# iris-ua/iris_lama

Hardware: AMD Instinct MI355X
Metric: particle-scans/sec (higher is better)
Workload: dtype f64; 1 GPU; PFSlam2D 30 particles, 1080-beam synthetic corridor log (SURVEY.md 8(d)), res 0.05 m, patch 32, l2_max 0.5, GN+Cauchy(0.15), seed 42; particles=30, beams=1080, parallelism=particle-shard x1

## Files before the change

iris_lama_amd/csrc/lama_dev.h:

```cpp
#pragma once
#include <hip/hip_runtime.h>
#include <stdint.h>
#include <cstddef>
#include <type_traits>

#ifdef LAMA_WIDE_DM
#define lama_dev lama_dev_wide
#endif

#include "lama_heap.h"

#ifdef LAMA_WAVE_SIM
#define LAMA_LOCKSTEP() ((void)__ballot(true))
#else
#define LAMA_LOCKSTEP() ((void)0)
#endif

namespace lama_dev {

#ifdef LAMA_WIDE_DM
typedef uint32_t sv_t;
constexpr uint32_t SV_VALID = 0x80000000u;
constexpr uint32_t SV_QUEUED = 0x40000000u;
constexpr uint32_t SV_SQMASK = 0x3FFFFFFFu;
constexpr int SV_VALID_BIT = 31;
constexpr uint32_t MAX_OFFSET_CELLS = 255;
#else
typedef uint16_t sv_t;
constexpr uint16_t SV_VALID = 0x8000;
constexpr uint16_t SV_QUEUED = 0x4000;
constexpr uint16_t SV_SQMASK = 0x3FFF;
constexpr int SV_VALID_BIT = 15;
constexpr uint32_t MAX_OFFSET_CELLS = 127;
#endif
constexpr uint32_t SV_BYTES = (uint32_t)sizeof(sv_t);
constexpr uint32_t SV_PATCH_BYTES = 1024u * SV_BYTES;

constexpr int ERR_WINDOW = 1;
constexpr int ERR_DM_CAP = 2;
constexpr int ERR_OCC_CAP = 4;
constexpr int ERR_QUEUE = 8;
constexpr int ERR_NUMERIC = 16;
constexpr int ERR_CLEAN_ABORT = 32;

struct Affine {
    double R[3][3];
    double t[3];
};

struct PartRec {
    uint32_t home, dm_cap, occ_cap, r0;
    sv_t* dm_sv; uint32_t* dm_obs; uint64_t* dm_mask;
    uint32_t* occ; uint64_t* occ_mask; uint64_t* occ_hit;
    int32_t* rev;
    uint64_t r1;
};

struct DevParams {
    uint32_t P;
    uint32_t W;
    uint32_t WC;
    uint32_t wx0, wy0;
    uint32_t qcap;
    const PartRec* part;
    uint32_t max_sqdist;
    uint32_t max_iter;
    double scale, off, resolution, maxdist, meas_sigma;
    double trunc_ray, trunc_range;
    int16_t* dm_dir;
    int16_t* occ_dir;
    int32_t* counts;
    double* poses;
    uint64_t* q_lower;
    uint64_t* q_raise;
    uint32_t* qsizes;
    uint32_t* slow;
    uint32_t* slow_list;
    uint32_t* slow_n;
    uint8_t* heavy;
    const uint32_t* elist;
    const uint32_t* elist_n;
    const uint8_t* early;
    uint32_t lane;
    uint64_t* act;
    uint32_t* act_count;
    uint32_t act_cap;
    uint64_t* stats;
    int32_t* err;
    uint64_t* dbg;
    uint32_t* guard;
    uint32_t guard_r;
    uint32_t occ_policy, ray_rule;
    uint32_t strategy;
    double lo_miss, lo_hit, lo_min, lo_max;
    uint32_t ghosts;
};

constexpr int ARG_BLOCK = 16;
struct PoseTable { double v[4 * ARG_BLOCK]; };
struct TfTable { double v[12 * ARG_BLOCK]; };
struct NoTable {};

struct PV {
    int16_t* dm_dir; int16_t* occ_dir;
    sv_t* dm_sv; uint32_t* dm_obs; uint64_t* dm_mask;
    uint32_t* occ; uint64_t* occ_mask; uint64_t* occ_hit;
    int32_t* counts; int32_t* rev;
    uint32_t dm_cap, occ_cap;
};
#ifdef LAMA_WAVE_SIM
__device__ inline uint32_t part_u32(const uint32_t* q) { return *q; }
__device__ inline uint64_t part_u64(const uint64_t* q) { return *q; }
#else
__device__ inline uint32_t part_u32(const uint32_t* q)
{
    return (uint32_t)__builtin_amdgcn_readfirstlane((int)__hip_atomic_load(q, __ATOMIC_RELAXED, __HIP_MEMORY_SCOPE_AGENT));
}
__device__ inline uint64_t part_u64(const uint64_t* q)
{
    const uint64_t v = __hip_atomic_load(q, __ATOMIC_RELAXED, __HIP_MEMORY_SCOPE_AGENT);
    const uint32_t lo = (uint32_t)__builtin_amdgcn_readfirstlane((int)(uint32_t)v), hi = (uint32_t)__builtin_amdgcn_readfirstlane((int)(uint32_t)(v >> 32));
    return ((uint64_t)hi << 32) | lo;
}
#endif
#if defined(LAMA_KC_PROBE) && !defined(LAMA_WAVE_SIM)
__device__ uint32_t g_kc_n;
__device__ uint64_t g_kc_ev[64][8];
__device__ __noinline__ void kc_probe(const DevParams& prm, int p)
{
    const uint64_t* q = reinterpret_cast<const uint64_t*>(prm.part + p);
#if LAMA_KC_PROBE == 2
    __builtin_amdgcn_s_dcache_inv();
#endif
    const unsigned long long act = __ballot(1);
    const bool rec = (int)(threadIdx.x & 63u) == __ffsll((long long)act) - 1;
    for (int k = 0; k < 9; ++k) {
        const uint64_t* qa = q + k;
        const uint64_t ua = (uint64_t)qa;
        const uint64_t sa = ((uint64_t)(uint32_t)__builtin_amdgcn_readfirstlane((int)(uint32_t)(ua >> 32)) << 32) | (uint32_t)__builtin_amdgcn_readfirstlane((int)(uint32_t)ua);
// ... 418 lines not shown
```

iris_lama_amd/csrc/lama_hip.hip:

```cpp
#include "../../include/lama_hip.h"

#include <hip/hip_runtime.h>

#include <algorithm>
#include <cmath>
#include <cstdio>
#include <cstdlib>
#include <cstring>
#include <map>
#include <memory>
#include <mutex>
#include <string>
#include <vector>

#include "lama_kernels.h"
#include "lama_pgo.h"
#include "lama_pgo_pcg.h"
#include "lama_map_build.h"
#include "lama_raster.h"
#include "lama_frontier.h"
#include "lama_raycast_query.h"
#include "lama_match_batch.h"
#include "lama_correlative.h"
#include "../host/pgo_pattern.hpp"
// ... 150 lines not shown
    size_t ev_used = 0;
    bool initialised = false;
    bool poisoned = false;
    bool dm_deleted = false;

    uint32_t P = 0, W = 0, WC = 0, wx0 = 0, wy0 = 0;
    uint32_t max_sqdist = 0;
    double scale = 0, off = 0;

    MapStore ms;
    std::vector<RegionAlloc> ra_dm, ra_occ;
    std::vector<HostPart> h_part;
    DevBuf<PartRec> d_part;
    PinVec<PartRec> h_part_stage;
    PinVec<CloneJob> h_jobs; DevBuf<CloneJob> d_jobs;
    PinVec<ZeroJob> h_zjobs; DevBuf<ZeroJob> d_zjobs;
    uint32_t floor_dm = 128, floor_occ = 128;
    PinVec<uint32_t> h_guard;
    uint64_t clone_bytes = 0;
    double* d_poses = nullptr;
    DevBuf<uint64_t> d_qlower, d_qraise;
    uint64_t* d_stats = nullptr;
    DevBuf<uint32_t> d_qsizes;
    DevBuf<uint64_t> d_dbg;
    DevBuf<uint32_t> d_slow;
    DevBuf<uint32_t> d_slow_list; uint32_t* d_slow_n = nullptr;
    DevBuf<uint8_t> d_heavy;
    DevBuf<uint8_t> d_early; DevBuf<uint32_t> d_elist;
    Stream stream3; Event ev_alloc, ev_go, ev_early;
    bool early_ok = false;
    uint32_t early_candidates = 0;
    std::vector<double> h_ll; bool ll_valid = false;
    PinVec<uint32_t> h_hlist; DevBuf<uint32_t> d_hlist;
    uint32_t early_on = 1;
    uint32_t early_min_count = 1024;
    Stream stream2; Event ev_route, ev_heavy;
    uint32_t route_min_count = 64, route_min_events = 48, route_percent = 150, route_cap = 64;
    bool route_forced = false; uint32_t num_cus = 256;
    bool debug_tail = false, debug_window = false;
    uint32_t big_stage_pad = 0;
    DevBuf<uint64_t> d_act; DevBuf<uint32_t> d_act_count;
    DevBuf<lama_dev::RayRec> d_rrec; DevBuf<uint64_t> d_rbbox; DevBuf<lama_dev::RayChunk> d_rchunk;
    int32_t* d_err = nullptr;
    DevBuf<double> d_pts; uint32_t last_n = 0;
    PinVec<uint64_t> h_stats;
    PinVec<double> h_tfs, h_pts;
    PinVec<int32_t> h_err;
    PinVec<uint32_t> h_slow_n;
    DevBuf<double> d_tfs;
    double* d_loglik = nullptr; int32_t* d_iters = nullptr;
    DevBuf<uint8_t> d_results;
    size_t results_bytes = 0, status_off = 0, status_bytes = 0;
    PinVec<uint8_t> h_status;
    PinVec<uint8_t> h_results;
    DevBuf<int32_t> d_oldcounts;
    DevBuf<double> d_mb_pts, d_mb_tfs; DevBuf<uint32_t> d_mb_offs; DevBuf<lama_dev::MbRay> d_mb_rays;
    DevBuf<uint32_t> d_mb_table, d_mb_off, d_mb_list, d_mb_bins; DevBuf<int32_t> d_mb_slot; DevBuf<uint64_t> d_mb_meta;
    PinVec<double> h_mb_tfs; PinVec<uint32_t> h_mb_offs; PinVec<uint64_t> h_mb_meta;
    DevBuf<uint8_t> d_raster; PinVec<uint8_t> h_raster;
    DevBuf<lama_dev::FrontierRec> d_frontier_rec;
    DevBuf<double> d_rq_in; DevBuf<uint8_t> d_rq_out; PinVec<double> h_rq_tfs;
    DevBuf<double> d_bposes, d_bout;
    DevBuf<double> d_msb_f64; DevBuf<uint32_t> d_msb_u32;
    PinVec<double> h_msb_f64; PinVec<uint32_t> h_msb_u32;
    DevBuf<double> d_cs_tfs; DevBuf<uint64_t> d_cs_best;
    PinVec<double> h_cs_tfs;

    double scan_reach = 0.0;
    uint32_t visit_bound = 0;
    DevBuf<uint32_t> d_scalar;
    DevBuf<lama_dev::ShipDesc> d_ship_desc; DevBuf<uint8_t> d_ship_heads;
    PinVec<lama_dev::ShipDesc> h_ship_desc; PinVec<uint8_t> h_ship_heads;
    uint32_t* d_guard = nullptr;
    Affine last_mtf; uint32_t last_first = 0, last_count = 0;
    bool last_guarded = false;
    int recover_depth = 0;
    int64_t mbx0 = 0, mbx1 = 0, mby0 = 0, mby1 = 0; bool mb_valid = false;
    bool unguarded_retry = false;
    uint32_t saved_visit_bound = 0; lama_hip_counters saved_ctr;
    bool pending_maps = false;
    StepGroup grp[MAX_STEP_GROUPS];
    Stream stream4;
    uint32_t step_groups = 1;
    uint32_t groups_ran = 0;
    std::vector<int32_t> deferred_idx; bool resample_deferred = false;
    bool groups_busy = false;
    PinVec<double> h_pts2; uint32_t scan_slot = 0;
    std::vector<uint64_t> h_chain;
    bool chain_dirty = false;
    double step_ms[3] = {0, 0, 0}; bool step_ms_any[3] = {false, false, false};
    PinVec<double> h_poses;
    PinVec<int32_t> h_counts;
    lama_hip_counters ctr;

    ~lama_hip_ctx()
    {
        (void)hipSetDevice(cfg.device);
        if (stream) (void)hipStreamSynchronize(stream);
        for (StepGroup& g : grp) if (g.s) (void)hipStreamSynchronize(g.s);
    }
};

namespace {

int32_t hip_fail(lama_hip_ctx* ctx, hipError_t e, const char* what)
{
    ctx->error = std::string(what) + ": " + hipGetErrorString(e);
    (void)hipStreamSynchronize(ctx->stream);
    if (ctx->groups_busy) for (StepGroup& g : ctx->grp) if (g.s) (void)hipStreamSynchronize(g.s);
    return LAMA_HIP_E_HIP;
}
#define HIPCHK(ctx, call)                                                                              \
    do {                                                                                               \
        const hipError_t e_ = (call);                                                                  \
        if (e_ != hipSuccess) return hip_fail((ctx), e_, #call);                                       \
    } while (0)

int32_t fail(lama_hip_ctx* ctx, int32_t code, const std::string& msg)
{
    ctx->error = msg;
    return code;
}

Affine moving_tf(const double* origin3, const double* q)
{
    Affine a;
    const double w = q ? q[0] : 1.0, x = q ? q[1] : 0.0, y = q ? q[2] : 0.0, z = q ? q[3] : 0.0;
    const double tx = 2.0 * x, ty = 2.0 * y, tz = 2.0 * z;
    const double twx = tx * w, twy = ty * w, twz = tz * w;
    const double txx = tx * x, txy = ty * x, txz = tz * x;
    const double tyy = ty * y, tyz = tz * y, tzz = tz * z;
    a.R[0][0] = 1.0 - (tyy + tzz); a.R[0][1] = txy - twz;         a.R[0][2] = txz + twy;
    a.R[1][0] = txy + twz;         a.R[1][1] = 1.0 - (txx + tzz); a.R[1][2] = tyz - twx;
    a.R[2][0] = txz - twy;         a.R[2][1] = tyz + twx;         a.R[2][2] = 1.0 - (txx + tyy);
    for (int i = 0; i < 3; ++i) a.t[i] = origin3 ? origin3[i] : 0.0;
    return a;
}

void host_scan_tf(const double* pose4, const Affine& m, double* out12)
{
    const double theta = std::atan2(pose4[1], pose4[0]);
    const double sn = std::sin(theta), cs = std::cos(theta);
    const double F[3][3] = {{cs, 0.0 - sn, 0.0}, {sn, cs, 0.0}, {0.0, 0.0, (1.0 - cs) + cs}};
    const double ft[3] = {pose4[2], pose4[3], 0.0};
    for (int i = 0; i < 3; ++i) {
        for (int j = 0; j < 3; ++j) out12[3 * i + j] = (F[i][0] * m.R[0][j] + F[i][1] * m.R[1][j]) + F[i][2] * m.R[2][j];
        out12[9 + i] = ((F[i][0] * m.t[0] + F[i][1] * m.t[1]) + F[i][2] * m.t[2]) + ft[i];
    }
}

uint32_t guard_radius(const lama_hip_ctx* c)
{
    const uint32_t r = (uint32_t)std::ceil(std::sqrt((double)c->max_sqdist));
    return ((c->dm_deleted ? 2u * r + 1u : r) + 1u + 31u) / 32u;
}

DevParams make_params(const lama_hip_ctx* c)
{
    DevParams p;
    p.P = c->P; p.W = c->W; p.WC = c->WC; p.wx0 = c->wx0; p.wy0 = c->wy0;
    p.qcap = c->cfg.queue_capacity; p.part = c->d_part;
    p.max_sqdist = c->max_sqdist; p.max_iter = c->cfg.max_iter;
    p.scale = c->scale; p.off = c->off; p.resolution = c->cfg.resolution;
    p.maxdist = std::sqrt((double)c->max_sqdist) * c->cfg.resolution;
    p.meas_sigma = c->cfg.meas_sigma;
    p.trunc_ray = c->cfg.truncated_ray; p.trunc_range = c->cfg.truncated_range;
// ... 18 lines not shown
}

int32_t wait_for_groups(lama_hip_ctx* c)
{
    if (!c->groups_busy) return LAMA_HIP_OK;
    for (StepGroup& g : c->grp)
        if (g.count) { const hipError_t e = hipStreamSynchronize(g.s); if (e != hipSuccess) { c->error = std::string("hipStreamSynchronize(group stream): ") + hipGetErrorString(e); return LAMA_HIP_E_HIP; } }
    return LAMA_HIP_OK;
}

bool scan_reach2(const double* pts, size_t n, bool strict, double& r2)
{
    double nan_acc = r2 = 0.0;
    for (size_t i = 0; i < n; ++i) { const double d2 = pts[3 * i] * pts[3 * i] + pts[3 * i + 1] * pts[3 * i + 1] + pts[3 * i + 2] * pts[3 * i + 2]; r2 = std::max(r2, d2); nan_acc += d2 * 0.0; }
    return std::isfinite(r2) && (!strict || nan_acc == 0.0);
}

int32_t upload_scan(lama_hip_ctx* c, const double* pts, uint32_t n)
{
    if (!pts) {
        if (c->last_n == 0 || n != c->last_n) return fail(c, LAMA_HIP_E_INVALID, "pts == NULL but no matching scan is resident");
        return LAMA_HIP_OK;
    }
    c->last_n = n;
    HIPCHK(c, c->d_pts.grow((size_t)3 * n, (size_t)3 * 2048));
    c->h_pts.resize((size_t)3 * n);
    std::memcpy(c->h_pts.data(), pts, sizeof(double) * 3 * n);
    double r2 = 0.0;
    if (!scan_reach2(pts, n, false, r2)) { c->last_n = 0; return fail(c, LAMA_HIP_E_INVALID, "the scan holds a non-finite point (filter NaN / inf ranges before the update, as iris_lama_ros does)"); }
    c->scan_reach = std::sqrt(r2);
    HIPCHK(c, hipMemcpyAsync(c->d_pts, c->h_pts.data(), sizeof(double) * 3 * n, hipMemcpyHostToDevice, c->stream));
    return LAMA_HIP_OK;
}

int32_t ensure_batch(lama_hip_ctx* c, size_t entries, size_t floor = 0)
{
    if (entries <= c->d_bout.n) return LAMA_HIP_OK;
    c->d_bposes.reset(); c->d_bout.reset();
    const size_t cap = std::max(entries, floor);
    HIPCHK(c, c->d_bposes.alloc(4 * cap));
    HIPCHK(c, c->d_bout.alloc(cap));
    return LAMA_HIP_OK;
}

void resolve_timers(lama_hip_ctx* c);
int32_t grow_arenas(lama_hip_ctx* c, uint32_t first, uint32_t count);
int32_t recover_update(lama_hip_ctx* c, int32_t e);
int32_t run_update_maps(lama_hip_ctx* c, uint32_t n, const Affine& mtf, uint32_t first, uint32_t count);
int32_t permute_particles(lama_hip_ctx* c, const int32_t* idx);

int32_t clamp_counts(lama_hip_ctx* c, bool fetch)
{
    if (fetch) HIPCHK(c, hipMemcpyAsync(c->h_counts.data(), c->ms.counts, sizeof(int32_t) * 2 * c->P, hipMemcpyDeviceToHost, c->stream));
    HIPCHK(c, hipStreamSynchronize(c->stream));
    bool clamped = false;
    for (uint32_t p = 0; p < c->P; ++p) {
        const HostPart& hp = c->h_part[p];
        if ((uint32_t)c->h_counts[2 * p] > hp.dm_cap) { c->h_counts[2 * p] = (int32_t)hp.dm_cap; clamped = true; }
        if ((uint32_t)c->h_counts[2 * p + 1] > hp.occ_cap) { c->h_counts[2 * p + 1] = (int32_t)hp.occ_cap; clamped = true; }
    }
    if (clamped) {
        HIPCHK(c, hipMemcpyAsync(c->ms.counts, c->h_counts.data(), sizeof(int32_t) * 2 * c->P, hipMemcpyHostToDevice, c->stream));
        HIPCHK(c, hipStreamSynchronize(c->stream));
    }
    return LAMA_HIP_OK;
}

int32_t device_error_result(lama_hip_ctx* c, int32_t e)
{
    if (e & ERR_WINDOW) return fail(c, LAMA_HIP_E_WINDOW, "a map cell fell outside the device window (the mapped area is wider than 1016 patches)");
    if (e & ERR_DM_CAP) return fail(c, LAMA_HIP_E_CAPACITY, "a particle's distance map exceeds 32767 patches (or the device is out of memory)");
    if (e & ERR_OCC_CAP) return fail(c, LAMA_HIP_E_CAPACITY, "a particle's occupancy map exceeds 32767 patches (or the device is out of memory)");
    if (e & ERR_QUEUE) return fail(c, LAMA_HIP_E_CAPACITY, "brushfire queue full (raise cfg.queue_capacity)");
    return fail(c, LAMA_HIP_E_NUMERIC, "unit complex number is (near) zero (SophusException in the reference)");
}

struct StatusView {
    const uint8_t *err, *slow_n, *stats, *guard, *counts; uint32_t base, n;
    int32_t error() const { int32_t e; std::memcpy(&e, err, sizeof(e)); return e; }
};

void apply_update_status(lama_hip_ctx* c, const StatusView& v, uint32_t first, uint32_t count, uint64_t* chain)
{
    uint32_t sn[5]; std::memcpy(sn, v.slow_n, sizeof(sn));
    c->ctr.brushfire_handovers += sn[0]; c->ctr.replay_handovers += sn[1] + sn[3]; c->ctr.brushfire_routed += sn[2] + sn[4]; c->ctr.brushfire_early += sn[4];
    c->early_candidates = sn[2] + sn[4];
    c->h_guard.resize(c->P);
    std::memcpy(&c->h_guard[v.base], v.guard, sizeof(uint32_t) * v.n);
    std::memcpy(&c->h_counts[2 * (size_t)v.base], v.counts, sizeof(int32_t) * 2 * v.n);
    if (v.error() != 0) return;
    for (uint32_t p = first; p < first + count; ++p) {
        uint64_t st[4]; std::memcpy(st, v.stats + sizeof(st) * (p - v.base), sizeof(st));
        c->ctr.ray_cells += st[2]; c->ctr.bf_cells += st[3]; if (chain) chain[p] = st[3];
    }
}

void refresh_patch_totals(lama_hip_ctx* c)
{
    c->ctr.dm_patches = c->ctr.occ_patches = 0;
    for (uint32_t p = 0; p < c->P; ++p) { c->ctr.dm_patches += c->h_counts[2 * p]; c->ctr.occ_patches += c->h_counts[2 * p + 1]; }
}

int32_t check_device_errors(lama_hip_ctx* c, bool maps = false, bool match = false, bool err_in_results = false)
{
    c->h_err.resize(1);
    int32_t& e = c->h_err[0] = 0;
    if (maps || match) c->h_stats.resize((size_t)c->P * 4);
    if (maps) {
        c->h_status.resize(c->status_bytes); c->h_slow_n.resize(5);
        HIPCHK(c, hipMemcpyAsync(c->h_status.data(), c->d_results + c->status_off, c->status_bytes, hipMemcpyDeviceToHost, c->stream));
    } else {
        if (match) {
            HIPCHK(c, hipMemcpyAsync(c->h_counts.data(), c->ms.counts, sizeof(int32_t) * 2 * c->P, hipMemcpyDeviceToHost, c->stream));
            HIPCHK(c, hipMemcpyAsync(c->h_stats.data(), c->d_stats, sizeof(uint64_t) * c->h_stats.size(), hipMemcpyDeviceToHost, c->stream));
        }
        if (!err_in_results) HIPCHK(c, hipMemcpyAsync(&e, c->d_err, sizeof(e), hipMemcpyDeviceToHost, c->stream));
    }
    HIPCHK(c, hipStreamSynchronize(c->stream));
    if (maps) {
        const uint8_t* const b = c->h_status.data(), * const sn = b + ((const uint8_t*)c->d_slow_n - (c->d_results + c->status_off));
        const StatusView v{b, sn, sn + 32, sn + 32 + 32 * (size_t)c->P, sn + 32 + 40 * (size_t)c->P, 0u, c->P};
        e = v.error();
        std::memcpy(c->h_slow_n.data(), v.slow_n, 5 * sizeof(uint32_t));
        std::memcpy(c->h_stats.data(), v.stats, sizeof(uint64_t) * 4 * c->P);
        apply_update_status(c, v, c->last_first, c->last_count, nullptr);
    }
    if (err_in_results) std::memcpy(&e, c->h_results.data() + ((const uint8_t*)c->d_err - c->d_results), sizeof(e));
    resolve_timers(c);
    if (e != 0) {
        HIPCHK(c, hipMemsetAsync(c->d_err, 0, sizeof(int32_t), c->stream));
        if (maps && (e & ERR_CLEAN_ABORT) && (e & (ERR_DM_CAP | ERR_OCC_CAP)) && !(e & ERR_WINDOW) && c->last_guarded && c->recover_depth < 10) {
            const int32_t rr = recover_update(c, e);
            if (rr != LAMA_HIP_E_CAPACITY) return rr;
        }
        if (e & (ERR_DM_CAP | ERR_OCC_CAP)) { const int32_t rcl = clamp_counts(c, !(maps || match)); if (rcl) return rcl; }
        return device_error_result(c, e);
    }
    if (match) for (uint32_t p = 0; p < c->P; ++p) { c->ctr.gn_iterations += c->h_stats[4 * p]; c->ctr.gn_evals += c->h_stats[4 * p + 1]; }
    if (maps || match) refresh_patch_totals(c);
    if (!maps) return LAMA_HIP_OK;
    uint64_t mx = 0, sum = 0; uint32_t arg = 0;
    for (uint32_t p = c->last_first; p < c->last_first + c->last_count; ++p) { const uint64_t v = c->h_stats[4 * p + 3]; sum += v; if (v > mx) { mx = v; arg = p; } }
    c->ctr.bf_longest_chain_sum += mx; c->ctr.bf_longest_chain_last = mx;
    if (c->debug_tail) {
        uint32_t rank = 0; double ll = 0, mean_ll = 0;
        if (c->h_results.size() >= c->results_bytes && c->P > 1) {
            const double* L = reinterpret_cast<const double*>(c->h_results.data() + sizeof(double) * 4 * c->P);
            ll = L[arg];
            for (uint32_t p = 0; p < c->P; ++p) { rank += L[p] < ll ? 1u : 0u; mean_ll += L[p]; }
            mean_ll /= c->P;
        }
        std::fprintf(stderr, "brushfire pops: mean %.0f max %llu (particle %u) handovers %u brushfire %.3f ms; log-lik of that particle %.1f (pool mean %.1f), rank %u of %u\n", (double)sum / c->P, (unsigned long long)mx, arg, c->h_slow_n[0], c->ctr.ms_brushfire, ll, mean_ll, rank, c->P);
    }
    return grow_arenas(c, 0, c->P);
}

constexpr uint32_t MAX_PATCHES = 32767u;

static uint32_t round_up32(uint32_t v) { return (v + 31u) / 32u * 32u; }

static uint32_t want_capacity(uint32_t floor_cap, uint32_t count, uint32_t extra)
{
    const uint32_t head = std::max<uint32_t>(std::max<uint32_t>(32u, count / 4u), extra);
    return std::min<uint32_t>(MAX_PATCHES, std::max<uint32_t>(floor_cap, round_up32(count + head)));
}

static PartRec dev_part(const lama_hip_ctx* c, const HostPart& h)
{
// ... 328 lines not shown
    const dim3 grid((unsigned)P, (unsigned)((std::max(WW, nWW) + 255) / 256));
    int16_t* const to_dm = nd[0]; int16_t* const to_occ = nd[1];
    hipLaunchKernelGGL(k_shift_window, grid, dim3(256), 0, c->stream, c->ms.dm_dir, to_dm, c->W, newW, dx, dy, WW, nWW, c->d_err);
    hipLaunchKernelGGL(k_shift_window, grid, dim3(256), 0, c->stream, c->ms.occ_dir, to_occ, c->W, newW, dx, dy, WW, nWW, c->d_err);
    {
        hipError_t e = hipGetLastError();
        if (e == hipSuccess) e = hipStreamSynchronize(c->stream);
        if (e != hipSuccess) return hip_fail(c, e, "k_shift_window");
    }
    c->ms.dm_dir.swap(nd[0]); c->ms.occ_dir.swap(nd[1]);
    if (newW != c->W) {
        c->W = newW; c->WC = newW * 32; c->cfg.window_patches = newW;
        c->ctr.window_growths += 1;
    }
    c->wx0 = (uint32_t)(nox * 32); c->wy0 = (uint32_t)(noy * 32);
    c->ctr.window_shifts += 1;
    c->ctr.window_patches = c->W;
    return LAMA_HIP_OK;
}

int32_t ensure_window(lama_hip_ctx* c, int64_t x0, int64_t x1, int64_t y0, int64_t y1)
{
    if (!c->mb_valid) { c->mbx0 = x0; c->mbx1 = x1; c->mby0 = y0; c->mby1 = y1; c->mb_valid = true; }
    else { c->mbx0 = std::min(c->mbx0, x0); c->mbx1 = std::max(c->mbx1, x1); c->mby0 = std::min(c->mby0, y0); c->mby1 = std::max(c->mby1, y1); }
    const int64_t ox = c->wx0 >> 5, oy = c->wy0 >> 5, W = c->W;
    if (c->debug_window) std::fprintf(stderr, "ensure_window: box x [%ld, %ld] y [%ld, %ld] mapped x [%ld, %ld] y [%ld, %ld] window x [%ld, %ld) y [%ld, %ld)\n", (long)x0, (long)x1, (long)y0, (long)y1, (long)c->mbx0, (long)c->mbx1, (long)c->mby0, (long)c->mby1, (long)ox, (long)(ox + W), (long)oy, (long)(oy + W));
    if (c->mbx0 >= ox && c->mbx1 < ox + W && c->mby0 >= oy && c->mby1 < oy + W) return LAMA_HIP_OK;
    const int64_t span = std::max(c->mbx1 - c->mbx0 + 1, c->mby1 - c->mby0 + 1);
    int64_t newW = W;
    if (span > W) newW = std::min<int64_t>(LAMA_HIP_MAX_WINDOW, std::max<int64_t>((span + 8 + 7) / 8 * 8, (W + W / 2 + 7) / 8 * 8));
    int64_t hx0 = c->mbx0, hx1 = c->mbx1, hy0 = c->mby0, hy1 = c->mby1;
    if (span > newW) { hx0 = x0; hx1 = x1; hy0 = y0; hy1 = y1; if (x1 - x0 + 1 > newW || y1 - y0 + 1 > newW) return LAMA_HIP_OK; }
    auto place = [&](int64_t o, int64_t lo, int64_t hi) {
        const int64_t a = hi - newW + 1, b = lo;
        int64_t no = std::min(std::max(o, a), b);
        if (no > o) no = std::min(no + 4, b); else if (no < o) no = std::max(no - 4, a);
        return no;
    };
    const int64_t nox = c->initialised ? place(ox, hx0, hx1) : (hx0 + hx1 + 1) / 2 - newW / 2;
    const int64_t noy = c->initialised ? place(oy, hy0, hy1) : (hy0 + hy1 + 1) / 2 - newW / 2;
    return regrid_window(c, (uint32_t)newW, nox, noy);
}

int32_t start_without_first_scan(lama_hip_ctx* c)
{
    if (c->initialised) return LAMA_HIP_OK;
    for (uint32_t p = 0; p < c->P; ++p) { c->h_poses[4 * p] = 1.0; c->h_poses[4 * p + 1] = 0.0; c->h_poses[4 * p + 2] = 0.0; c->h_poses[4 * p + 3] = 0.0; }
    HIPCHK(c, hipMemcpyAsync(c->d_poses, c->h_poses.data(), sizeof(double) * 4 * c->P, hipMemcpyHostToDevice, c->stream));
    c->initialised = true;
    return LAMA_HIP_OK;
}

int32_t fit_window(lama_hip_ctx* c, const Affine& mtf, uint32_t first, uint32_t count)
{
    double far = c->scan_reach;
    if (c->cfg.ray_rule == 0 && c->cfg.truncated_range > 0.0) far = std::min(far, c->cfg.truncated_range);
    const uint32_t guard_r = guard_radius(c);
    const double reach = far + std::sqrt(mtf.t[0] * mtf.t[0] + mtf.t[1] * mtf.t[1]) + (double)(guard_r + 1u) * 32.0 * c->cfg.resolution;
    double xlo = 1e300, xhi = -1e300, ylo = 1e300, yhi = -1e300;
    for (uint32_t p = first; p < first + count; ++p) {
        const double x = c->h_poses[4 * p + 2], y = c->h_poses[4 * p + 3];
        xlo = std::min(xlo, x - reach); xhi = std::max(xhi, x + reach);
        ylo = std::min(ylo, y - reach); yhi = std::max(yhi, y + reach);
    }
    auto patch = [&](double w) { return (int64_t)std::floor((c->scale * w + c->off) / 32.0); };
    return ensure_window(c, patch(xlo), patch(xhi), patch(ylo), patch(yhi));
}

static uint32_t route_places(const lama_hip_ctx* c, uint32_t count)
{
    const uint32_t slots = c->num_cus * 12u;
    if (c->route_forced || count >= slots) return c->route_cap;
    return std::min<uint32_t>(c->route_cap, std::max<uint32_t>(8u, (slots - count) / 7u));
}

struct UpdatePlan {
    hipStream_t s = nullptr; const double* d_pts = nullptr; uint32_t n = 0, first = 0, count = 0;
    DevParams prm;
    lama_dev::TfTable tab = lama_dev::TfTable(); bool tf_by_value = false;
    StepGroup* timers = nullptr;
    bool sequential = false, guarded = true, canon = false, two_waves = false, route = false, early_lane = false;
    bool prev_routed = false; uint32_t host_n = 0;
    uint32_t route_places = 0; unsigned gy = 0, resume_grid = 0; bool replay_large = true;
};

static bool parallel_raycast_ruled_out(const lama_hip_ctx* c, uint32_t n)
{
    return c->cfg.sequential_raycast == 1 || c->cfg.occupancy_policy == 1 || c->cfg.ray_rule == 1 || n > 4096u || (uint64_t)n + 4096u > c->cfg.active_capacity;
}

UpdatePlan plan_update(lama_hip_ctx* c, uint32_t n, uint32_t first, uint32_t count, bool wrap_sequential, StepGroup* g = nullptr)
{
    UpdatePlan u;
    u.n = n; u.first = first; u.count = count; u.timers = g; u.tf_by_value = g && count <= (uint32_t)lama_dev::ARG_BLOCK;
    u.s = g ? g->s : (hipStream_t)c->stream; u.d_pts = g ? (const double*)g->d_pts : (const double*)c->d_pts; u.prm = g ? group_params(c, *g) : make_params(c);
    u.two_waves = c->cfg.brushfire_waves == 2 || (c->cfg.brushfire_waves == 0 && count <= BF_TW_MAX_PARTICLES);
    u.gy = count <= 64 ? 128u : (count >= 1024 ? 8u : 32u);
#ifdef LAMA_WAVE_SIM
    u.gy = 4u;
#endif
    u.replay_large = count <= 512; u.resume_grid = std::min<unsigned>(count, 256u);
    if (g) return u;
    u.sequential = parallel_raycast_ruled_out(c, n) || wrap_sequential;
    u.guarded = c->cfg.ray_rule == 0;
    u.canon = c->cfg.brushfire_mode == 1;
    u.route = u.two_waves && count >= c->route_min_count && c->route_cap > 0; u.route_places = route_places(c, count);
    if (u.sequential || !(c->early_on && u.two_waves && !u.canon && first == 0 && count == c->P &&
                          count >= std::max<uint32_t>(c->route_min_count, c->early_min_count) && c->route_cap > 0)) return u;
    if (c->ll_valid) {
        double mean = 0; for (uint32_t p = 0; p < c->P; ++p) mean += c->h_ll[p]; mean /= c->P;
        const double lim = 2.5 * std::min(mean, 0.0) - 5.0;
        std::vector<std::pair<double, uint32_t>> cand;
        for (uint32_t p = 0; p < c->P; ++p) if (c->h_ll[p] < lim) cand.emplace_back(c->h_ll[p], p);
        if (cand.size() > u.route_places) { std::partial_sort(cand.begin(), cand.begin() + u.route_places, cand.end()); cand.resize(u.route_places); }
        c->h_hlist.resize(256);
        for (auto& e : cand) c->h_hlist[u.host_n++] = e.second;
    }
    u.prev_routed = c->early_ok && c->early_candidates > 0; u.early_lane = u.host_n > 0 || u.prev_routed;
    return u;
}

int32_t wrap_guard_probe(lama_hip_ctx* c, uint32_t n, int64_t& bound)
{
    if (parallel_raycast_ruled_out(c, n) || (uint64_t)c->visit_bound + n < 65536u) return LAMA_HIP_OK;
    uint32_t m = 0;
    if (c->initialised) {
        const DevParams prm = make_params(c);
        (void)hipMemsetAsync(c->d_scalar, 0, sizeof(uint32_t), c->stream);
        hipLaunchKernelGGL(k_occ_max_visited, dim3(c->P), dim3(256), 0, c->stream, prm, c->d_scalar);
        HIPCHK(c, hipMemcpyAsync(&m, c->d_scalar, sizeof(uint32_t), hipMemcpyDeviceToHost, c->stream));
        HIPCHK(c, hipStreamSynchronize(c->stream));
    }
    bound = m;
    return LAMA_HIP_OK;
}

int32_t pregrow_unguarded(lama_hip_ctx* c, uint32_t first, uint32_t count)
{
    if (c->cfg.ray_rule == 0) return LAMA_HIP_OK;
    const double rp = c->scan_reach / (32.0 * c->cfg.resolution) + 2.5;
    const uint32_t bound = (uint32_t)std::min(32767.0, std::ceil(3.1416 * rp * rp));
    std::vector<CapRequest> reqs;
    for (uint32_t p = first; p < first + count; ++p) {
        const HostPart& pr = c->h_part[p];
        const uint32_t nd = std::min<uint32_t>(MAX_PATCHES, round_up32((uint32_t)c->h_counts[2 * p] + bound)), no = std::min<uint32_t>(MAX_PATCHES, round_up32((uint32_t)c->h_counts[2 * p + 1] + bound));
        if (nd > pr.dm_cap || no > pr.occ_cap) reqs.push_back(CapRequest{p, std::max(nd, pr.dm_cap), std::max(no, pr.occ_cap)});
    }
    return reqs.empty() ? LAMA_HIP_OK : set_capacities(c, reqs);
}

void note_update_begin(lama_hip_ctx* c, const Affine& mtf, const UpdatePlan& u, int64_t probed)
{
    c->last_mtf = mtf; c->last_first = u.first; c->last_count = u.count; c->last_guarded = u.guarded;
    if (c->recover_depth == 0) { c->saved_visit_bound = c->visit_bound; c->saved_ctr = c->ctr; }
    if (probed >= 0) { c->visit_bound = (uint32_t)probed; if (u.sequential) c->ctr.wrap_guard_scans += 1; }
    c->visit_bound = (uint32_t)std::min<uint64_t>((uint64_t)c->visit_bound + u.n, 65535u);
    if (u.sequential) c->ctr.sequential_raycast_scans += 1; else c->ctr.parallel_raycast_scans += 1;
    c->early_ok = u.route && u.first == 0 && u.count == c->P;
}

int32_t stage_scan_tfs(lama_hip_ctx* c, const Affine& mtf, uint32_t first, uint32_t count, hipStream_t s, lama_dev::TfTable* tab)
{
    PinVec<double>& tfs = c->h_tfs; tfs.resize((size_t)c->P * 12);
    for (uint32_t p = first; p < first + count; ++p) host_scan_tf(&c->h_poses[4 * p], mtf, &tfs[12 * (size_t)p]);
    if (tab) std::memcpy(tab->v, &tfs[12 * (size_t)first], sizeof(double) * 12 * count);
    else HIPCHK(c, hipMemcpyAsync(c->d_tfs + 12 * (size_t)first, &tfs[12 * (size_t)first], sizeof(double) * 12 * count, hipMemcpyHostToDevice, s));
    return LAMA_HIP_OK;
}

static unsigned xcd_grid(const lama_hip_ctx* c, uint32_t first, uint32_t count)
{
    return first + count == c->P ? (count + 7u) / 8u * 8u : count;
}

template <class Tab>
int32_t launch_allocation_phase(lama_hip_ctx* c, const UpdatePlan& u, int alloc_only, const Tab& tab)
{
    const uint32_t n = u.n, first = u.first, count = u.count;
    const double* const d_tfs = u.tf_by_value ? nullptr : (const double*)c->d_tfs;
    const size_t need = (size_t)c->P * n;
    if (need > c->d_rrec.n) {
        c->d_rrec.reset(); c->d_rbbox.reset(); c->d_rchunk.reset();
        hipError_t e = c->d_rrec.alloc(need);
        if (e == hipSuccess) e = c->d_rbbox.alloc(need);
        if (e == hipSuccess) e = c->d_rchunk.alloc((size_t)c->P * ((n + 63) / 64));
        if (e != hipSuccess) { c->d_rrec.reset(); return hip_fail(c, e, "ray buffers"); }
    }
    const dim3 hits_grid(xcd_grid(c, first, count), (n + 255) / 256);
    hipLaunchKernelGGL(k_ray_hits<Tab>, hits_grid, dim3(256), 0, u.s, u.prm, u.d_pts, (int)n, d_tfs, (int)first,
                       (lama_dev::RayRec*)c->d_rrec, (uint64_t*)c->d_rbbox, alloc_only, (lama_dev::RayChunk*)c->d_rchunk, tab);
    const int rw_seg = count <= 64 ? 4 : 1;
    hipLaunchKernelGGL(k_ray_alloc_walk, dim3(xcd_grid(c, first, count), (n * rw_seg + 255) / 256), dim3(256), 0, u.s, u.prm, (const lama_dev::RayRec*)c->d_rrec, (int)n, (int)first, rw_seg);
    double far = c->scan_reach;
    if (c->cfg.truncated_range > 0.0) far = std::min(far, c->cfg.truncated_range);
    const int reach_cells = (int)std::ceil(far * c->scale) + 2;
    uint32_t row0 = 0, row1 = c->W - 1;
    if (c->mb_valid) {
        const int64_t oy = c->wy0 >> 5, W = c->W;
        const int64_t lo = std::min(std::max(c->mby0 - oy, (int64_t)0), W - 1), hi = std::min(std::max(c->mby1 - oy, (int64_t)0), W - 1);
        if (hi >= lo) { row0 = (uint32_t)lo; row1 = (uint32_t)hi; }
    }
    hipLaunchKernelGGL(k_occ_reverse_dir<Tab>, dim3(count), dim3(256), 0, u.s, u.prm, (int)first, d_tfs, reach_cells, c->unguarded_retry ? 1 : 0, row0, row1, tab);
    return LAMA_HIP_OK;
}
int32_t launch_allocation_phase(lama_hip_ctx* c, const UpdatePlan& u, int alloc_only) { return u.tf_by_value ? launch_allocation_phase(c, u, alloc_only, u.tab) : launch_allocation_phase(c, u, alloc_only, lama_dev::NoTable()); }

int32_t launch_early_lane(lama_hip_ctx* c, const UpdatePlan& u)
{
    DevParams pe = u.prm; pe.elist = c->d_elist; pe.elist_n = c->d_slow_n + 4; pe.lane = 1;
    hipLaunchKernelGGL(k_ray_patches, dim3(u.route_places, 128u), dim3(256), 0, c->stream, pe, (const lama_dev::RayRec*)c->d_rrec,
                       (const uint64_t*)c->d_rbbox, (const lama_dev::RayChunk*)c->d_rchunk, (int)u.n, 0);
    hipLaunchKernelGGL((k_ray_replay<RP_SORT_SMALL, RP_SORT_SMALL, false, RP_BLOCK_LARGE>), dim3(u.route_places), dim3(RP_BLOCK_LARGE), 0, c->stream, pe, 0);
    hipLaunchKernelGGL((k_ray_replay<8192, 8192, true, RP_BLOCK_LARGE>), dim3(u.route_places), dim3(RP_BLOCK_LARGE), 0, c->stream, pe, 0);
    HIPCHK(c, hipEventRecord(c->ev_alloc, c->stream));
    HIPCHK(c, hipStreamWaitEvent(c->stream3, c->ev_alloc, 0));
    hipLaunchKernelGGL(k_mark_early, dim3(1), dim3(64), 0, c->stream3, pe);
    HIPCHK(c, hipEventRecord(c->ev_go, c->stream3));
    hipLaunchKernelGGL((k_brushfire<LQ_BIG, RQ_BIG, true, true>), dim3(u.route_places), dim3(2 * UM_BLOCK), c->big_stage_pad, c->stream3, pe, 0, 2);
    HIPCHK(c, hipEventRecord(c->ev_early, c->stream3));
    HIPCHK(c, hipStreamWaitEvent(c->stream, c->ev_go, 0));
    return LAMA_HIP_OK;
}

int32_t launch_parallel_raycast(lama_hip_ctx* c, const UpdatePlan& u)
{
    const int first = (int)u.first; const uint32_t host_n = u.host_n;
    if (u.early_lane) {
        if (host_n) HIPCHK(c, hipMemcpyAsync(c->d_hlist, c->h_hlist.data(), sizeof(uint32_t) * host_n, hipMemcpyHostToDevice, c->stream));
        hipLaunchKernelGGL(k_early_list, dim3(1), dim3(256), 0, c->stream, u.prev_routed ? (const uint8_t*)c->d_heavy : (const uint8_t*)nullptr,
                           (const uint32_t*)c->d_hlist, host_n, c->d_early, c->d_elist, c->d_slow_n + 4, (int)c->P, u.route_places);
    }
    { const int32_t ra = launch_allocation_phase(c, u, 0); if (ra) return ra; }
    DevParams prm = u.prm;
    if (u.early_lane) { const int32_t re = launch_early_lane(c, u); if (re) return re; prm.early = c->d_early; }
    hipLaunchKernelGGL(k_ray_patches, dim3(xcd_grid(c, u.first, u.count), u.gy), dim3(256), 0, u.s, prm, (const lama_dev::RayRec*)c->d_rrec,
                       (const uint64_t*)c->d_rbbox, (const lama_dev::RayChunk*)c->d_rchunk, (int)u.n, first);
    if (u.replay_large) {
        hipLaunchKernelGGL((k_ray_replay<RP_SORT_SMALL, RP_SORT_SMALL, false, RP_BLOCK_LARGE>), dim3(u.count), dim3(RP_BLOCK_LARGE), 0, u.s, prm, first);
        hipLaunchKernelGGL((k_ray_replay<8192, 8192, true, RP_BLOCK_LARGE>), dim3(u.resume_grid), dim3(RP_BLOCK_LARGE), 0, u.s, prm, first);
    } else {
        hipLaunchKernelGGL((k_ray_replay<RP_SORT_SMALL, RP_SORT_SMALL, false, RP_BLOCK_SMALL>), dim3(u.count), dim3(RP_BLOCK_SMALL), 0, u.s, prm, first);
        hipLaunchKernelGGL((k_ray_replay<8192, 8192, true, RP_BLOCK_SMALL>), dim3(u.resume_grid), dim3(RP_BLOCK_SMALL), 0, u.s, prm, first);
    }
    return LAMA_HIP_OK;
}

int32_t launch_brushfire(lama_hip_ctx* c, const UpdatePlan& u)
{
    const int first = (int)u.first;
    DevParams prm = u.prm; if (u.early_lane) prm.early = c->d_early;
    if (u.canon) hipLaunchKernelGGL(k_brushfire_canon, dim3(u.count), dim3(CN_BLOCK), 0, u.s, prm, first);
    if (u.route) {
        prm.heavy = c->d_heavy;
        hipLaunchKernelGGL(k_bf_route, dim3(1), dim3(256), 0, c->stream, prm, first, (int)u.count, c->route_min_events, c->route_percent, u.route_places);
        HIPCHK(c, hipEventRecord(c->ev_route, c->stream));
        hipLaunchKernelGGL((k_brushfire<LQ_BIG, RQ_BIG, true, true>), dim3(u.route_places), dim3(2 * UM_BLOCK), 0, c->stream, prm, first, 1);
        HIPCHK(c, hipStreamWaitEvent(c->stream2, c->ev_route, 0));
        hipLaunchKernelGGL((k_brushfire<LQ_SMALL, RQ_SMALL, false, true>), dim3(u.count), dim3(2 * UM_BLOCK), 0, c->stream2, prm, first, 0);
        HIPCHK(c, hipEventRecord(c->ev_heavy, c->stream2));
        HIPCHK(c, hipStreamWaitEvent(c->stream, c->ev_heavy, 0));
    } else if (u.two_waves) hipLaunchKernelGGL((k_brushfire<LQ_SMALL, RQ_SMALL, false, true>), dim3(u.count), dim3(2 * UM_BLOCK), 0, u.s, prm, first, 0);
    else hipLaunchKernelGGL((k_brushfire<LQ_SMALL, RQ_SMALL, false, false>), dim3(u.count), dim3(UM_BLOCK), 0, u.s, prm, first, 0);
    if (u.two_waves) hipLaunchKernelGGL((k_brushfire<LQ_BIG, RQ_BIG, true, true>), dim3(u.resume_grid), dim3(2 * UM_BLOCK), 0, u.s, prm, first, 0);
    else hipLaunchKernelGGL((k_brushfire<LQ_BIG, RQ_BIG, true, false>), dim3(u.resume_grid), dim3(UM_BLOCK), 0, u.s, prm, first, 0);
    if (u.early_lane) HIPCHK(c, hipStreamWaitEvent(c->stream, c->ev_early, 0));
    hipLaunchKernelGGL(k_brushfire_slow, dim3(u.count), dim3(UM_BLOCK), 0, u.s, prm, first);
    return LAMA_HIP_OK;
}

int32_t launch_update(lama_hip_ctx* c, const UpdatePlan& u, Timer& ray_timer)
{
    int32_t rc = !u.sequential ? launch_parallel_raycast(c, u) : u.guarded ? launch_allocation_phase(c, u, 1) : LAMA_HIP_OK;
    if (rc) return rc;
    if (u.sequential) hipLaunchKernelGGL(k_raycast, dim3(u.count), dim3(UM_BLOCK), 0, u.s, u.prm, u.d_pts, (int)u.n, c->d_tfs, (int)u.first);
    ray_timer.stop();
    HIPCHK(c, hipGetLastError());
    Timer t = Timer::of_update(c, u.timers, 2);
    c->ctr.brushfire_mode = c->cfg.brushfire_mode; c->ctr.brushfire_waves = u.two_waves ? 2u : 1u;
    rc = launch_brushfire(c, u);
    if (rc) return rc;
    t.stop();
    HIPCHK(c, hipGetLastError());
    return LAMA_HIP_OK;
}

int32_t run_update_maps(lama_hip_ctx* c, uint32_t n, const Affine& mtf, uint32_t first, uint32_t count)
{
    int32_t rc = fit_window(c, mtf, first, count);
    if (rc == LAMA_HIP_OK) rc = stage_scan_tfs(c, mtf, first, count, c->stream, nullptr);
    if (rc) return rc;
    Timer t = Timer::of_update(c, nullptr, 1);
    const bool whole = first == 0 && count == c->P;
    (void)hipMemsetAsync(c->d_slow_n, 0, whole ? 32 + sizeof(uint64_t) * 4 * c->P : 32, c->stream);
    if (!whole) (void)hipMemsetAsync(c->d_stats + 4 * (size_t)first, 0, sizeof(uint64_t) * 4 * count, c->stream);
    int64_t probed = -1; rc = wrap_guard_probe(c, n, probed);
    if (rc == LAMA_HIP_OK) rc = pregrow_unguarded(c, first, count);
    if (rc) return rc;
    const UpdatePlan u = plan_update(c, n, first, count, probed >= 0 && (uint64_t)probed + n >= 65536u);
    note_update_begin(c, mtf, u, probed);
    return launch_update(c, u, t);
}


int32_t permute_particles(lama_hip_ctx* c, const int32_t* idx)
{
    const uint32_t P = c->P;
    std::vector<uint8_t> taken(P, 0);
    std::vector<HostPart> np(P);
    std::vector<int32_t> nc(2 * (size_t)P);
    std::vector<double> npose(4 * (size_t)P);
    std::vector<uint32_t> clones;
    for (uint32_t i = 0; i < P; ++i) {
        const uint32_t j = (uint32_t)idx[i];
        std::memcpy(&npose[4 * i], &c->h_poses[4 * j], sizeof(double) * 4);
        nc[2 * i] = c->h_counts[2 * j]; nc[2 * i + 1] = c->h_counts[2 * j + 1];
        if (!taken[j]) { taken[j] = 1; np[i] = c->h_part[j]; } else clones.push_back(i);
    }
    std::vector<uint32_t> dead;
    for (uint32_t j = 0; j < P; ++j) if (!taken[j]) dead.push_back(j);
    c->h_jobs.resize(0); c->h_zjobs.resize(0);
    c->clone_bytes = 0;
    const size_t WW = (size_t)c->W * c->W;
    uint32_t dir_off16 = 0, dir_n16 = (uint32_t)(WW * 2 / 16);
    {
        const int64_t oy = c->wy0 >> 5, W = c->W;
        if (c->mb_valid) {
            const int64_t lo = std::min(std::max(c->mby0 - oy, (int64_t)0), W - 1), hi = std::min(std::max(c->mby1 - oy, (int64_t)0), W - 1);
            if (hi >= lo) { dir_off16 = (uint32_t)(lo * W * 2 / 16); dir_n16 = (uint32_t)((hi - lo + 1) * W * 2 / 16); }
        }
    }
    struct Slot { bool keep_dm, keep_occ; HostPart rec; int32_t odm, oocc; };
    std::vector<Slot> slots(dead.size());
    for (size_t k = 0; k < dead.size(); ++k) {
        const uint32_t d = dead[k], i = clones[k], j = (uint32_t)idx[i];
        const HostPart& dr = c->h_part[d];
        const HostPart& sr = c->h_part[j];
        Slot sl{dr.dm_cap == sr.dm_cap, dr.occ_cap == sr.occ_cap, dr, c->h_counts[2 * d], c->h_counts[2 * d + 1]};
        void* dp[5];
        region_ptrs(c, dr, dp);
        ZeroJob z{};
        if (!sl.keep_dm) { z.ndm = sl.odm; z.d[0] = dp[0]; z.d[1] = dp[1]; z.d[2] = dp[2]; region_release(c, true, dr.dm_chunk, dr.dm_off, dr.dm_cap); }
        if (!sl.keep_occ) { z.nocc = sl.oocc; z.d[3] = dp[3]; z.d[4] = dp[4]; region_release(c, false, dr.occ_chunk, dr.occ_off, dr.occ_cap); }
        if (z.ndm || z.nocc) { c->h_zjobs.resize(c->h_zjobs.size() + 1); c->h_zjobs[c->h_zjobs.size() - 1] = z; }
        slots[k] = sl;
    }
// ... 252 lines not shown
        (cfg.window_patches & 7) || cfg.dm_patch_capacity > 32767 || cfg.occ_patch_capacity > 32767 ||
        cfg.queue_capacity < (uint32_t)LQ_BIG)
        return LAMA_HIP_E_INVALID;
    int ndev = 0;
    if (hipGetDeviceCount(&ndev) != hipSuccess || ndev <= 0 || cfg.device < 0 || cfg.device >= ndev) return LAMA_HIP_E_HIP;

    std::unique_ptr<lama_hip_ctx, Delete> owner(new lama_hip_ctx());
    lama_hip_ctx* c = owner.get();
    c->cfg = cfg;
    std::memset(&c->ctr, 0, sizeof(c->ctr));
    c->P = cfg.particles; c->W = cfg.window_patches; c->WC = c->W * 32;
    c->ctr.window_patches = c->W;
    c->debug_tail = std::getenv("LAMA_HIP_DEBUG_TAIL") != nullptr;
    c->debug_window = std::getenv("LAMA_HIP_DEBUG_WINDOW") != nullptr;
    {
        constexpr uint32_t CU_LDS = 160u * 1024u, GRAN = 1280u;
        const uint32_t used = (uint32_t)((sizeof(lama_dev::BfLds<LQ_BIG, RQ_BIG>) + GRAN - 1) / GRAN * GRAN);
        c->big_stage_pad = CU_LDS > used + 2u * GRAN ? CU_LDS - used - 2u * GRAN : 0u;
    }
    if (const char* rr = std::getenv("LAMA_HIP_BF_ROUTE")) {
        unsigned a = 0, b = 0, pc = 0, d = 0, e = 1;
        if (std::sscanf(rr, "%u,%u,%u,%u,%u", &a, &b, &pc, &d, &e) >= 4) { c->route_min_count = a; c->route_min_events = b; c->route_percent = pc; c->route_cap = std::min(d, 256u); c->early_on = e; c->early_min_count = 0; c->route_forced = true; }
    }
    c->scale = 1.0 / cfg.resolution;
    c->off = double(2642244ull >> 1) * 32.0;
    uint32_t md = (uint32_t)std::ceil(cfg.l2_max * c->scale);
    c->max_sqdist = md * md;
    if (c->max_sqdist == 0 || md > MAX_OFFSET_CELLS) return LAMA_HIP_E_INVALID;

    if (hipSetDevice(cfg.device)) return LAMA_HIP_E_HIP;
    { hipDeviceProp_t prop; if (hipGetDeviceProperties(&prop, cfg.device) == hipSuccess && prop.multiProcessorCount > 0) c->num_cus = (uint32_t)prop.multiProcessorCount; }
    if (hipStreamCreate(&c->stream.h) || hipEventCreate(&c->ev0.h) || hipEventCreate(&c->ev1.h)) return LAMA_HIP_E_HIP;
    const size_t P = c->P, WW = (size_t)c->W * c->W, dc = cfg.dm_patch_capacity, oc = cfg.occ_patch_capacity;
    {
        MapStore& m = c->ms;
        c->floor_dm = (uint32_t)dc; c->floor_occ = (uint32_t)oc;
        if (P * dc > 0xFFFFFFF0ull || P * oc > 0xFFFFFFF0ull) return LAMA_HIP_E_INVALID;
        if (m.dm_dir.alloc(P * WW) || hipMemset(m.dm_dir, 0xFF, P * WW * 2)) return LAMA_HIP_E_HIP;
        if (m.occ_dir.alloc(P * WW) || hipMemset(m.occ_dir, 0xFF, P * WW * 2)) return LAMA_HIP_E_HIP;
        if (add_chunk(c, true, (uint32_t)(P * dc)) != LAMA_HIP_OK || add_chunk(c, false, (uint32_t)(P * oc)) != LAMA_HIP_OK) return LAMA_HIP_E_HIP;
        c->ctr.pool_growths = 0;
        c->h_part.resize(P);
        for (size_t p = 0; p < P; ++p) {
            HostPart r{};
            r.home = (uint32_t)p; r.dm_cap = (uint32_t)dc; r.occ_cap = (uint32_t)oc;
            if (region_alloc(c, true, (uint32_t)dc, r.dm_chunk, r.dm_off) != LAMA_HIP_OK || region_alloc(c, false, (uint32_t)oc, r.occ_chunk, r.occ_off) != LAMA_HIP_OK) return LAMA_HIP_E_HIP;
            c->h_part[p] = r;
        }
        if (c->d_part.alloc(P)) return LAMA_HIP_E_HIP;
        if (upload_part(c) != LAMA_HIP_OK) return LAMA_HIP_E_HIP;
        if (hipStreamSynchronize(c->stream)) return LAMA_HIP_E_HIP;
    }
    c->results_bytes = P * 4 * 8 + P * 8 + P * 4 + 8;
    c->status_off = P * 4 * 8 + P * 8 + P * 4;
    const size_t slow_off = (c->results_bytes + 7) / 8 * 8;
    c->status_bytes = (slow_off - c->status_off) + 32 + P * 4 * 8 + P * 2 * 4 + P * 2 * 4;
    if (c->d_results.alloc(c->status_off + c->status_bytes) || hipMemset(c->d_results, 0, c->status_off + c->status_bytes)) return LAMA_HIP_E_HIP;
    c->d_poses = reinterpret_cast<double*>(c->d_results.p);
    c->d_loglik = c->d_poses + P * 4;
    c->d_iters = reinterpret_cast<int32_t*>(c->d_loglik + P);
    c->d_err = c->d_iters + P;
    c->d_slow_n = reinterpret_cast<uint32_t*>(c->d_results + slow_off);
    c->d_stats = reinterpret_cast<uint64_t*>(c->d_results + slow_off + 32);
    c->d_guard = reinterpret_cast<uint32_t*>(c->d_stats + P * 4);
    c->ms.counts = reinterpret_cast<int32_t*>(c->d_guard + P * 2);
    if (c->d_qlower.alloc(P * (size_t)cfg.queue_capacity) || c->d_qraise.alloc(P * (size_t)cfg.queue_capacity)) return LAMA_HIP_E_HIP;
    if (c->d_qsizes.alloc(P * 2) || hipMemset(c->d_qsizes, 0, P * 2 * 4)) return LAMA_HIP_E_HIP;
    if (c->d_dbg.alloc(P * 16 + (1u << 20) / 8) || hipMemset(c->d_dbg, 0, P * 16 * 8 + (1u << 20))) return LAMA_HIP_E_HIP;
    if (c->d_slow.alloc(P) || hipMemset(c->d_slow, 0, P * 4)) return LAMA_HIP_E_HIP;
    if (c->d_slow_list.alloc(4 * P) || hipMemset(c->d_slow_list, 0, 4 * P * 4)) return LAMA_HIP_E_HIP;
    if (c->d_heavy.alloc(P) || hipMemset(c->d_heavy, 0, P)) return LAMA_HIP_E_HIP;
    if (c->d_early.alloc(P) || hipMemset(c->d_early, 0, P)) return LAMA_HIP_E_HIP;
    if (c->d_elist.alloc(256) || hipMemset(c->d_elist, 0, 256 * 4)) return LAMA_HIP_E_HIP;
    if (c->d_hlist.alloc(256) || hipMemset(c->d_hlist, 0, 256 * 4)) return LAMA_HIP_E_HIP;
    if (hipStreamCreate(&c->stream2.h) || hipStreamCreate(&c->stream3.h)) return LAMA_HIP_E_HIP;
    {
        uint32_t G = c->P < c->route_min_count ? DEFAULT_STEP_GROUPS : 1u;
        if (const char* sg = std::getenv("LAMA_HIP_STEP_GROUPS")) {
            unsigned v = 0;
            if (std::sscanf(sg, "%u", &v) == 1 && v >= 1) G = std::min<uint32_t>(v, MAX_STEP_GROUPS);
        }
        if (c->P >= c->route_min_count) G = 1;
        c->step_groups = G;
        if (G > 1) {
            if (G > 3 && hipStreamCreate(&c->stream4.h)) return LAMA_HIP_E_HIP;
            const hipStream_t ss[MAX_STEP_GROUPS] = {c->stream, c->stream2, c->stream3, c->stream4};
            uint32_t per = (uint32_t)((P + G - 1) / G);
            const uint32_t per8 = (per + 7u) / 8u * 8u;
            if ((P + per8 - 1) / per8 == G) per = per8;
            for (uint32_t k = 0; k < G; ++k) {
                StepGroup& g = c->grp[k];
                g.s = ss[k];
                g.first = (uint32_t)std::min<size_t>(P, (size_t)k * per); g.count = (uint32_t)std::min<size_t>(P, (size_t)(k + 1) * per) - g.first;
                if (g.count == 0) continue;
                const GroupPack L(g.count);
                if (g.d_words.alloc(16) || hipMemset(g.d_words, 0, 64) || g.d_slow_list.alloc(4 * P) || hipMemset(g.d_slow_list, 0, 4 * P * 4) ||
                    g.d_pack.alloc(L.bytes) || hipEventCreateWithFlags(&g.ev_match.h, hipEventDisableTiming))
                    return LAMA_HIP_E_HIP;
                g.h_pack.resize(L.bytes);
                if (cfg.profile) for (Event& e : g.tev) if (hipEventCreate(&e.h)) return LAMA_HIP_E_HIP;
            }
            c->h_chain.assign(P, 0);
        }
    }
    if (hipEventCreateWithFlags(&c->ev_alloc.h, hipEventDisableTiming) || hipEventCreateWithFlags(&c->ev_early.h, hipEventDisableTiming) ||
        hipEventCreateWithFlags(&c->ev_go.h, hipEventDisableTiming) ||
        hipEventCreateWithFlags(&c->ev_route.h, hipEventDisableTiming) || hipEventCreateWithFlags(&c->ev_heavy.h, hipEventDisableTiming))
        return LAMA_HIP_E_HIP;
    if (c->d_scalar.alloc(4) || hipMemset(c->d_scalar, 0, 16)) return LAMA_HIP_E_HIP;
    if (c->d_act.alloc(P * (size_t)cfg.active_capacity)) return LAMA_HIP_E_HIP;
    if (c->d_act_count.alloc(P) || hipMemset(c->d_act_count, 0, P * 4)) return LAMA_HIP_E_HIP;
    if (c->d_tfs.alloc(P * 12) || c->d_oldcounts.alloc(P * 2)) return LAMA_HIP_E_HIP;
    if (hipDeviceSynchronize()) return LAMA_HIP_E_HIP;
    c->h_poses.assign(P * 4, 0.0);
    c->h_counts.assign(P * 2, 0);
    *out = owner.release();
    return LAMA_HIP_OK;
}

void lama_hip_ctx_destroy(lama_hip_ctx* c) { delete c; }

int32_t lama_hip_pf_set_poses(lama_hip_ctx* c, const double* poses)
{
    if (!c || !poses) return LAMA_HIP_E_INVALID;
    ENTER(c);
    HIPCHK(c, hipSetDevice(c->cfg.device));
    std::memcpy(c->h_poses.data(), poses, sizeof(double) * 4 * c->P);
    HIPCHK(c, hipMemcpyAsync(c->d_poses, c->h_poses.data(), sizeof(double) * 4 * c->P, hipMemcpyHostToDevice, c->stream));
    return LAMA_HIP_OK;
}

int32_t lama_hip_pf_get_poses(lama_hip_ctx* c, double* poses)
{
    if (!c || !poses) return LAMA_HIP_E_INVALID;
    ENTER(c);
    std::memcpy(poses, c->h_poses.data(), sizeof(double) * 4 * c->P);
    return LAMA_HIP_OK;
}

int32_t lama_hip_pf_init(lama_hip_ctx* c, const double* pts, uint32_t n, const double* origin3, const double* quat,
                         const double* pose0)
{
    if (!c || !pts || !pose0 || n == 0) return LAMA_HIP_E_INVALID;
    ENTER(c);
    if (c->initialised) return fail(c, LAMA_HIP_E_STATE, "lama_hip_pf_init called twice");
    HIPCHK(c, hipSetDevice(c->cfg.device));
    const double mx = c->scale * pose0[2] + c->off, my = c->scale * pose0[3] + c->off;
    const uint32_t px = ((uint32_t)mx) >> 5, py = ((uint32_t)my) >> 5;
    c->wx0 = (px - c->W / 2) * 32;
    c->wy0 = (py - c->W / 2) * 32;
    for (uint32_t p = 0; p < c->P; ++p) std::memcpy(&c->h_poses[4 * p], pose0, sizeof(double) * 4);
    HIPCHK(c, hipMemcpyAsync(c->d_poses, c->h_poses.data(), sizeof(double) * 4 * c->P, hipMemcpyHostToDevice, c->stream));
    int32_t rc = upload_scan(c, pts, n);
    if (rc) return rc;
    const Affine mtf = moving_tf(origin3, quat);
    rc = run_update_maps(c, n, mtf, 0, 1);
    if (rc) return rc;
    rc = check_device_errors(c, true, false);
    if (rc) return rc;
    if (c->P > 1) {
        std::vector<int32_t> idx(c->P, 0);
        rc = permute_particles(c, idx.data());
        if (rc) return rc;
    }
    rc = check_device_errors(c, true, false);
    if (rc) return rc;
// ... 847 lines not shown
    if (iterations) *iterations = st.iters;
    if (rel_residual_sq) *rel_residual_sq = st.bb == 0.0 ? 0.0 : st.rr / st.bb;
    if (outcome) *outcome = oc;
    if (model_decrease) *model_decrease = st.model;
    if (kernel_ms) { float ms = 0; PGOCHK(g, hipEventElapsedTime(&ms, g->ev0, g->ev1)); *kernel_ms = ms; }
    return LAMA_HIP_OK;
}

int32_t lama_hip_pgo_try_solved_step(lama_hip_pgo* g, double* half_chi2, double* kernel_ms)
{
    if (!g || !half_chi2) return LAMA_HIP_E_INVALID;
    if (!g->solution_valid) {
        g->error = "lama_hip_pgo_try_solved_step: no solution of the system at the current state (call lama_hip_pgo_solve_pcg first)";
        return LAMA_HIP_E_STATE;
    }
    g->candidate_pending = false;
    PGOCHK(g, hipSetDevice(g->device));
    PgoPtrs p{g->d_cand, g->d_fi, g->d_fj, g->d_meas, g->d_sqrt, g->d_err, g->d_hoff, g->d_fdi, g->d_fdj, g->d_fg, g->d_incptr, g->d_inc,
              g->d_hdiag, g->d_b, g->d_chi};
    PGOCHK(g, hipEventRecord(g->ev0, g->stream));
    hipLaunchKernelGGL(k_pgo_retract, dim3((g->N + PGO_BLOCK - 1) / PGO_BLOCK), dim3(PGO_BLOCK), 0, g->stream, (const double*)g->d_poses,
                       (const double*)g->d_px, (double*)g->d_cand, g->N);
    if (g->robust) hipLaunchKernelGGL(k_pgo_error_robust, dim3(g->blocksF), dim3(PGO_BLOCK), 0, g->stream, p, pgo_loss_ptrs(g), (const double*)g->d_cand, g->F);
    else hipLaunchKernelGGL(k_pgo_error, dim3(g->blocksF), dim3(PGO_BLOCK), 0, g->stream, p, (const double*)g->d_cand, g->F);
    hipLaunchKernelGGL(k_pgo_sum, dim3(1), dim3(64), 0, g->stream, (const double*)g->d_chi, g->blocksF, (double*)g->d_half);
    PGOCHK(g, hipEventRecord(g->ev1, g->stream));
    PGOCHK(g, hipGetLastError());
    double h = 0.0;
    PGOCHK(g, hipMemcpyAsync(&h, g->d_half, sizeof(double), hipMemcpyDeviceToHost, g->stream));
    PGOCHK(g, hipStreamSynchronize(g->stream));
    *half_chi2 = h;
    g->candidate_pending = true;
    if (kernel_ms) { float ms = 0; PGOCHK(g, hipEventElapsedTime(&ms, g->ev0, g->ev1)); *kernel_ms = ms; }
    return LAMA_HIP_OK;
}

int32_t lama_hip_map_add_obstacles(lama_hip_ctx* c, uint32_t particle, const uint32_t* cells_xy, uint32_t n)
{
    if (!c || !cells_xy || n == 0 || particle >= c->P) return LAMA_HIP_E_INVALID;
    ENTER(c);
    HIPCHK(c, hipSetDevice(c->cfg.device));
    {
        const int64_t r = (int64_t)guard_radius(c);
        int64_t x0 = INT64_MAX, x1 = INT64_MIN, y0 = INT64_MAX, y1 = INT64_MIN;
        for (uint32_t i = 0; i < n; ++i) {
            const int64_t px = cells_xy[2 * i] >> 5, py = cells_xy[2 * i + 1] >> 5;
            x0 = std::min(x0, px); x1 = std::max(x1, px); y0 = std::min(y0, py); y1 = std::max(y1, py);
        }
        const int32_t rw = ensure_window(c, x0 - r, x1 + r, y0 - r, y1 + r);
        if (rw) return rw;
    }
    { const int32_t rf = start_without_first_scan(c); if (rf) return rf; }
    {
        const int r = (int)guard_radius(c);
        std::vector<uint64_t> keys;
        keys.reserve((size_t)n);
        uint64_t last = ~0ull;
        for (uint32_t i = 0; i < n; ++i) {
            const uint64_t k = ((uint64_t)(cells_xy[2 * i + 1] >> 5) << 32) | (uint64_t)(cells_xy[2 * i] >> 5);
            if (k != last) { keys.push_back(k); last = k; }
        }
        std::sort(keys.begin(), keys.end());
        keys.erase(std::unique(keys.begin(), keys.end()), keys.end());
        std::vector<uint64_t> dil;
        dil.reserve(keys.size() * (size_t)((2 * r + 1) * (2 * r + 1)));
        for (uint64_t k : keys)
            for (int dy = -r; dy <= r; ++dy)
                for (int dx = -r; dx <= r; ++dx) dil.push_back((((k >> 32) + (uint64_t)(int64_t)dy) << 32) | (uint32_t)((uint32_t)k + (uint32_t)dx));
        std::sort(dil.begin(), dil.end());
        dil.erase(std::unique(dil.begin(), dil.end()), dil.end());
        const uint64_t want = (uint64_t)c->h_counts[2 * particle] + dil.size();
        if (want > c->h_part[particle].dm_cap) {
            const int32_t rg = set_capacities(c, {CapRequest{particle, (uint32_t)std::min<uint64_t>(MAX_PATCHES, (want + 31u) / 32u * 32u), c->h_part[particle].occ_cap}});
            if (rg) return rg;
        }
        c->last_guarded = false;
    }
    DevBuf<uint32_t> cells;
    HIPCHK(c, cells.alloc(2 * (size_t)n));
    uint32_t* const d_cells = cells;
    HIPCHK(c, hipMemcpyAsync(d_cells, cells_xy, sizeof(uint32_t) * 2 * (size_t)n, hipMemcpyHostToDevice, c->stream));
    DevParams prm = make_params(c);
    if (n > c->cfg.queue_capacity) return fail(c, LAMA_HIP_E_CAPACITY, "more obstacle cells than cfg.queue_capacity");
    HIPCHK(c, hipMemsetAsync(c->d_slow_n, 0, 5 * sizeof(uint32_t), c->stream));
    hipLaunchKernelGGL(k_dm_add_obstacles, dim3(1), dim3(UM_BLOCK), 0, c->stream, prm, (int)particle, d_cells, n);
    hipLaunchKernelGGL((k_brushfire<LQ_SMALL, RQ_SMALL, false, true>), dim3(1), dim3(2 * UM_BLOCK), 0, c->stream, prm, (int)particle, 0);
    hipLaunchKernelGGL((k_brushfire<LQ_BIG, RQ_BIG, true, true>), dim3(1), dim3(2 * UM_BLOCK), 0, c->stream, prm, (int)particle, 0);
    hipLaunchKernelGGL(k_brushfire_slow, dim3(1), dim3(UM_BLOCK), 0, c->stream, prm, (int)particle);
    HIPCHK(c, hipGetLastError());
    c->last_first = 0; c->last_count = c->P;
    return check_device_errors(c, true, false);
}

int32_t lama_hip_map_integrate_scans(lama_hip_ctx* c, uint32_t particle, uint32_t K, const double* poses4, const double* pts, const uint32_t* offs,
                                     const double* origins, const double* quats, uint32_t flags)
{
    if (!c || particle >= c->P || (flags & ~3u)) return LAMA_HIP_E_INVALID;
    ENTER(c);
    if (c->cfg.occupancy_policy != 0) return fail(c, LAMA_HIP_E_INVALID, "key scans are integrated into a frequency occupancy map (cfg.occupancy_policy 0)");
    if (K == 0) return LAMA_HIP_OK;
    if (!poses4 || !offs) return fail(c, LAMA_HIP_E_INVALID, "poses4 / scan_offsets missing");
    for (uint32_t k = 0; k < K; ++k)
        if (offs[k + 1] < offs[k]) return fail(c, LAMA_HIP_E_INVALID, "scan_offsets must not decrease");
    const uint64_t total64 = (uint64_t)offs[K] - offs[0];
    if (total64 == 0) return LAMA_HIP_OK;
    if (!pts || total64 >= (uint64_t)MB_HIT) return fail(c, LAMA_HIP_E_INVALID, "pts_xyz missing, or more than 2^31 - 1 points");
    const uint32_t total = (uint32_t)total64;
    const bool full = flags & 1u, prune = flags & 2u;
    c->h_mb_tfs.resize((size_t)12 * K); c->h_mb_offs.resize((size_t)K + 1);
    for (uint32_t k = 0; k < K; ++k) {
        host_scan_tf(poses4 + 4 * (size_t)k, moving_tf(origins ? origins + 3 * (size_t)k : nullptr, quats ? quats + 4 * (size_t)k : nullptr), &c->h_mb_tfs[12 * (size_t)k]);
        for (int j = 0; j < 12; ++j)
            if (!std::isfinite(c->h_mb_tfs[12 * (size_t)k + j])) return fail(c, LAMA_HIP_E_INVALID, "a key pose or sensor transform is not finite");
    }
    for (uint32_t k = 0; k <= K; ++k) c->h_mb_offs[k] = offs[k] - offs[0];
    HIPCHK(c, hipSetDevice(c->cfg.device));
    HIPCHK(c, c->d_mb_pts.grow((size_t)3 * total)); HIPCHK(c, c->d_mb_tfs.grow((size_t)12 * K)); HIPCHK(c, c->d_mb_offs.grow((size_t)K + 1));
    HIPCHK(c, c->d_mb_rays.grow(total)); HIPCHK(c, c->d_mb_meta.grow(8));
    c->h_mb_meta.resize(8);
    MbBounds* const d_bounds = reinterpret_cast<MbBounds*>(c->d_mb_meta.p);
    MbMeta* const d_meta = reinterpret_cast<MbMeta*>(c->d_mb_meta.p + 4);
    {
        MbBounds b0{0xFFFFFFFFu, 0u, 0xFFFFFFFFu, 0u, 0u, 0u, 0ull};
        std::memcpy(c->h_mb_meta.data(), &b0, sizeof(b0));
    }
    HIPCHK(c, hipMemcpyAsync(c->d_mb_meta, c->h_mb_meta.data(), sizeof(MbBounds), hipMemcpyHostToDevice, c->stream));
    HIPCHK(c, hipMemcpyAsync(c->d_mb_pts, pts + 3 * (size_t)offs[0], sizeof(double) * 3 * total, hipMemcpyHostToDevice, c->stream));
    HIPCHK(c, hipMemcpyAsync(c->d_mb_tfs, c->h_mb_tfs.data(), sizeof(double) * 12 * K, hipMemcpyHostToDevice, c->stream));
    HIPCHK(c, hipMemcpyAsync(c->d_mb_offs, c->h_mb_offs.data(), sizeof(uint32_t) * ((size_t)K + 1), hipMemcpyHostToDevice, c->stream));
    auto untruncated_params = [c]() { DevParams p = make_params(c); p.trunc_ray = 0.0; p.trunc_range = 0.0; return p; };
    DevParams prm = untruncated_params();
    const unsigned ray_blocks = (total + 255u) / 256u;
    MbRay* const d_rays = c->d_mb_rays;
    {
        Timer t(c, &c->ctr.ms_raycast, &c->ctr.launches_raycast);
        hipLaunchKernelGGL(k_mb_geom, dim3(ray_blocks), dim3(256), 0, c->stream, prm, (const double*)c->d_mb_pts, (const uint32_t*)c->d_mb_offs,
                           (const double*)c->d_mb_tfs, K, total, full ? 1 : 0, d_rays, d_bounds);
        t.stop();
    }
    HIPCHK(c, hipGetLastError());
    HIPCHK(c, hipMemcpyAsync(c->h_mb_meta.data(), c->d_mb_meta, sizeof(MbBounds), hipMemcpyDeviceToHost, c->stream));
    HIPCHK(c, hipStreamSynchronize(c->stream));
    MbBounds bnd;
    std::memcpy(&bnd, c->h_mb_meta.data(), sizeof(bnd));
    if (bnd.flags & MB_NONFINITE) { resolve_timers(c); return fail(c, LAMA_HIP_E_INVALID, "a key scan holds a non-finite point (filter NaN / inf ranges first, as iris_lama_ros does)"); }
    if (bnd.flags & MB_TOO_LONG) { resolve_timers(c); return fail(c, LAMA_HIP_E_WINDOW, "a ray is longer than 8191 cells"); }
    {
        const int64_t x0 = bnd.x0, x1 = bnd.x1, y0 = bnd.y0, y1 = bnd.y1;
        const int64_t ux0 = c->mb_valid ? std::min(c->mbx0, x0) : x0, ux1 = c->mb_valid ? std::max(c->mbx1, x1) : x1;
        const int64_t uy0 = c->mb_valid ? std::min(c->mby0, y0) : y0, uy1 = c->mb_valid ? std::max(c->mby1, y1) : y1;
        if (ux1 - ux0 + 1 > LAMA_HIP_MAX_WINDOW || uy1 - uy0 + 1 > LAMA_HIP_MAX_WINDOW) {
            resolve_timers(c);
            return fail(c, LAMA_HIP_E_WINDOW, "the key scans and the map so far are wider than the largest device window (1016 patches)");
        }
        const int32_t rw = ensure_window(c, x0, x1, y0, y1);
        if (rw) { resolve_timers(c); return rw; }
    }
    { const int32_t rf = start_without_first_scan(c); if (rf) return rf; }
    const uint32_t bx0 = bnd.x0 - (c->wx0 >> 5), by0 = bnd.y0 - (c->wy0 >> 5), bw = bnd.x1 - bnd.x0 + 1u, bh = bnd.y1 - bnd.y0 + 1u, nb = bw * bh;
    if (bx0 + bw > c->W || by0 + bh > c->W) { resolve_timers(c); return fail(c, LAMA_HIP_E_WINDOW, "the key scans fell outside the device window"); }
    HIPCHK(c, c->d_mb_table.grow(nb)); HIPCHK(c, c->d_mb_off.grow((size_t)nb + 1)); HIPCHK(c, c->d_mb_list.grow(nb)); HIPCHK(c, c->d_mb_slot.grow(nb));
    prm = untruncated_params();
    uint32_t* const d_table = c->d_mb_table; uint32_t* const d_off = c->d_mb_off; uint32_t* const d_list = c->d_mb_list; int32_t* const d_slot = c->d_mb_slot;
    HIPCHK(c, hipMemsetAsync(d_table, 0, sizeof(uint32_t) * nb, c->stream));
    {
        Timer t(c, &c->ctr.ms_raycast, &c->ctr.launches_raycast);
        hipLaunchKernelGGL(k_mb_bin, dim3(ray_blocks), dim3(256), 0, c->stream, prm, (const MbRay*)d_rays, total, bx0, by0, bw, bh, d_table, (const uint32_t*)nullptr, (uint32_t*)nullptr);
// ... 869 lines not shown
```

iris_lama_amd/csrc/lama_kernels.h:

```cpp
#pragma once
#include "lama_dev.h"

namespace lama_dev {

constexpr int SM_BLOCK = 256;
constexpr int UM_BLOCK = 64;
#ifdef LAMA_TEST_SMALL_QUEUES
constexpr int LQ_SMALL = LAMA_TEST_SMALL_QUEUES, RQ_SMALL = LAMA_TEST_SMALL_QUEUES / 4;
#else
constexpr int LQ_SMALL = 1024, RQ_SMALL = 256;
#endif
constexpr int LQ_BIG = 8192, RQ_BIG = 2048;
constexpr uint32_t BF_TW_MAX_PARTICLES = 1u << 30;

template <int CTRL, int ROW_MASK>
__device__ __forceinline__ double dpp_add(double v)
{
    const uint64_t u = (uint64_t)__double_as_longlong(v);
    const uint32_t lo = (uint32_t)__builtin_amdgcn_update_dpp(0, (int)(uint32_t)u, CTRL, ROW_MASK, 0xF, false);
    const uint32_t hi = (uint32_t)__builtin_amdgcn_update_dpp(0, (int)(uint32_t)(u >> 32), CTRL, ROW_MASK, 0xF, false);
    return v + __longlong_as_double((long long)(((uint64_t)hi << 32) | lo));
}

template <int NV>
// ... 921 lines not shown
__device__ __forceinline__ void lds_push_flat(uint64_t* heap, uint32_t& n, const uint64_t* ent, const uint32_t* cnt_p, const int lane, uint64_t* dummy)
{
    const uint32_t l4 = (uint32_t)lane & 3u;
    const uint64_t entry = ent[l4];
    const uint32_t pos = n + l4;
    const uint32_t pprio = heap_prio(heap[n >= 4 ? (pos - 1) / 2 : 0]);
    const uint32_t cnt_v = *cnt_p;
    const bool mine = (uint32_t)lane < cnt_v;
    const bool up = mine && pprio > heap_prio(entry);
    const unsigned long long upm = __ballot(up);
    const uint32_t cnt = (uint32_t)__builtin_amdgcn_readfirstlane((int)cnt_v);
    if (cnt == 0) return;
    if (__builtin_expect(n >= 4 && upm == 0ull, 1)) {
        uint64_t* dst = mine ? heap + pos : dummy;
        *dst = entry;
        n += cnt;
        LAMA_LOCKSTEP();
        return;
    }
    #pragma unroll 1
    for (uint32_t i = 0; i < cnt; ++i) lds_push(heap, n, ent[i], lane == 0);
}

__device__ __forceinline__ void lds_push_flat_n(uint64_t* heap, uint32_t& n, const uint64_t* ent, const uint32_t cnt, const int lane, uint64_t* dummy)
{
    if (cnt == 0) return;
    const uint32_t l4 = (uint32_t)lane & 3u;
    const uint64_t entry = ent[l4];
    const uint32_t pos = n + l4;
    const uint32_t pprio = heap_prio(heap[n >= 4 ? (pos - 1) / 2 : 0]);
    const bool mine = (uint32_t)lane < cnt;
    const bool up = mine && pprio > heap_prio(entry);
    const unsigned long long upm = __ballot(up);
    if (n >= 4 && upm == 0ull) {
        uint64_t* dst = mine ? heap + pos : dummy;
        *dst = entry;
        n += cnt;
        LAMA_LOCKSTEP();
        return;
    }
    #pragma unroll 1
    for (uint32_t i = 0; i < cnt; ++i) lds_push(heap, n, ent[i], lane == 0);
}

__device__ __forceinline__ bool lds_push_list(uint64_t* heap, uint32_t& n, const uint64_t* ent, const uint32_t cnt, int lane)
{
    if (!cnt) return false;
    const uint32_t l4 = (uint32_t)lane & 3u;
    const uint64_t entry = ent[l4];
    const uint32_t pos = n + l4;
    if (n >= 4) {
        const uint32_t pprio = heap_prio(heap[(pos - 1) / 2]);
        const bool mine = (uint32_t)lane < cnt;
        const bool up = mine && pprio > heap_prio(entry);
        if (__ballot(up) == 0) {
            if (mine) heap[pos] = entry;
            n += cnt;
            LAMA_LOCKSTEP();
            return true;
        }
    }
    #pragma unroll 1
    for (uint32_t i = 0; i < cnt; ++i) lds_push(heap, n, ent[i], lane == 0);
    return false;
}

#ifdef LAMA_WAVE_SIM
__device__ __forceinline__ void lds_barrier() { __syncthreads(); }
#else
__device__ __forceinline__ void lds_barrier() { asm volatile("s_waitcnt lgkmcnt(0)\n\ts_barrier" ::: "memory"); }
#endif

#ifdef LAMA_WAVE_SIM
__device__ __forceinline__ uint64_t uniform_u64(uint64_t v) { return v; }
#else
__device__ __forceinline__ uint64_t uniform_u64(uint64_t v)
{
    return ((uint64_t)(uint32_t)__builtin_amdgcn_readfirstlane((int)(uint32_t)(v >> 32)) << 32) | (uint32_t)__builtin_amdgcn_readfirstlane((int)(uint32_t)v);
}
#endif

__device__ __forceinline__ void bf_hand_over(const DevParams& prm, int p, bool from_resume)
{
    prm.slow[p] = 1;
    if (!from_resume) prm.slow_list[atomicAdd(prm.slow_n, 1u)] = (uint32_t)p;
}

template <int LQ_LDS, int RQ_LDS, bool RESUME, bool TW>
__device__ __forceinline__ void bf_particle(const DevParams& prm, const int p_any, BfLds<LQ_LDS, RQ_LDS>& sh)
{
    const int p = __builtin_amdgcn_readfirstlane(p_any);
    if (!RESUME && prm.heavy != nullptr && (prm.heavy[p] != 0 || (prm.early != nullptr && prm.early[p] != 0))) return;
    const uint32_t handed = RESUME ? prm.slow[p] : 1u;
    const int lane = threadIdx.x & 63;
    const int tid = threadIdx.x, nthreads = TW ? 2 * UM_BLOCK : UM_BLOCK;
    const PV pv = pview_w(prm, p);
    int16_t* dir = pv.dm_dir;
    sv_t* sv = pv.dm_sv;
    uint32_t* obs = pv.dm_obs;
    uint64_t* mask = pv.dm_mask;
    const uint32_t dm_cap = pv.dm_cap;
    uint64_t* g_lower = prm.q_lower + (size_t)p * prm.qcap;
    uint64_t* g_raise = prm.q_raise + (size_t)p * prm.qcap;
    int count = uload_i32(prm.counts + 2 * p);
    const uint64_t nlr = uload_u64(prm.qsizes + 2 * p);
    uint32_t nl = (uint32_t)nlr, nr = (uint32_t)(nlr >> 32);
    if (RESUME && TW) __syncthreads(); else LAMA_LOCKSTEP();
    if (RESUME && handed == 0) return;
    if (tid == 0) prm.slow[p] = 0;
    if (nl == 0 && nr == 0) return;
    if (nl + 4 > (uint32_t)LQ_LDS || nr + 4 > (uint32_t)RQ_LDS) { if (tid == 0) bf_hand_over(prm, p, RESUME); return; }

    for (int k = tid; k < DC_SIZE; k += nthreads) sh.dc[k] = DC_EMPTY;
    for (uint32_t k = tid; k < nl; k += nthreads) sh.lower[k] = g_lower[k];
    for (uint32_t k = tid; k < nr; k += nthreads) sh.raise[k] = g_raise[k];
    __syncthreads();
    const uint64_t anc = lds_pop_ancestors(lane);
    constexpr uint32_t LOWER_CAP = RESUME ? (uint32_t)LQ_LDS : (uint32_t)(LQ_LDS + RQ_LDS);
#ifndef LAMA_WAVE_SIM
    if (TW) { if (tid >= UM_BLOCK) __builtin_amdgcn_s_setprio(0); else __builtin_amdgcn_s_setprio(3); }
#endif
    if (TW && tid >= UM_BLOCK) {
        __syncthreads();
        uint32_t hnl = (uint32_t)__builtin_amdgcn_readfirstlane((int)sh.cmd), hnr = (uint32_t)__builtin_amdgcn_readfirstlane((int)sh.cmd_r);
        if (hnl == BF_CMD_EXIT) return;
#ifdef LAMA_PROFILE_BF
        uint64_t hp[3] = {0, 0, 0};
        uint64_t ht = __builtin_readcyclecounter();
        #define HFT(k) do { const uint64_t t_ = __builtin_readcyclecounter(); hp[k] += t_ - ht; ht = t_; } while (0)
#else
        #define HFT(k) do {} while (0)
#endif
        constexpr int NR = LQ_LDS > 2047 ? 3 : 2;
        #define BF_HELPER_POP(H, N, B) do { if (NR == 3 && (N) > 2047u) lds_pop_flat<3>(H, N, lane, anc, &sh.topq[B], dmy); else lds_pop_flat<2>(H, N, lane, anc, &sh.topq[B], dmy); } while (0)
        uint64_t* const dmy = sh.dummy[1] + (lane & (BF_DUMMY - 1));
        uint32_t it = 0;
        bool hstop = false;
        while (hnr > 0) {
            const uint32_t b = it & 1u;
            BF_HELPER_POP(sh.raise, hnr, b);
            lds_barrier();
            lds_push_flat(sh.raise, hnr, sh.pr_e[b], &sh.pr_n[b], lane, dmy);
            lds_push_flat(sh.lower, hnl, sh.pl_e[b], &sh.pl_n[b], lane, dmy);
            ++it;
            if (hnl + 4 > (uint32_t)LQ_LDS || (hnr > 0 && hnr + 4 > (uint32_t)RQ_LDS) || (hnr == 0 && hnl == 0)) { hstop = true; break; }
            if (hnr == 0) lds_barrier();
        }
        if (!hstop && hnl > 0) for (;;) {
            const uint32_t b = it & 1u;
            BF_HELPER_POP(sh.lower, hnl, b);
            HFT(0);
            lds_barrier();
            HFT(1);
            lds_push_flat(sh.lower, hnl, sh.pl_e[b], &sh.pl_n[b], lane, dmy);
            HFT(2);
            ++it;
            if (hnl - 1u >= LOWER_CAP - 4u) break;
        }
#ifdef LAMA_PROFILE_BF
#ifndef LAMA_PROFILE_BF_MAIN
        if (lane == 0) for (int k = 0; k < 3; ++k) prm.dbg[8 * p + 5 + k] = hp[k];
#endif
#endif
        #undef HFT
        #undef BF_HELPER_POP
        __syncthreads();
        return;
    }
    const DirCache dc{sh.dc, dir, prm.W};
    const bool ghosts = prm.ghosts != 0u;
    auto obstacle_get = [&](const bool want, const int gx, const int gy) {
        const bool in = (uint32_t)gx < prm.WC && (uint32_t)gy < prm.WC;
        if (want && !in) atomicOr(prm.err, ERR_WINDOW);
        const bool w = want && in;
        if (!__ballot(w)) return;
        const uint32_t gpidx = ((uint32_t)gy >> 5) * prm.W + ((uint32_t)gx >> 5);
        const uint32_t gci = ((uint32_t)gx & 31u) | (((uint32_t)gy & 31u) << 5);
        const int gs = coop_slot(dc, dir, count, (int)dm_cap, w, gpidx, ERR_DM_CAP, prm.err);
        if (w && gs >= 0) atomicOr((unsigned long long*)(mask + (size_t)gs * 16 + (gci >> 6)), 1ull << (gci & 63));
    };

    const int ddx = lane == 0 ? 1 : (lane == 2 ? -1 : 0), ddy = lane == 1 ? 1 : (lane == 3 ? -1 : 0);
    const bool is_cur = lane == 4, is_nb = lane < 4;
    uint64_t processed = 0;
    bool spill = false;
#ifdef LAMA_PROFILE_BF
    uint64_t prof[8] = {0, 0, 0, 0, 0, 0, 0, 0};
    uint64_t tprev = __builtin_readcyclecounter();
#endif

    #define BF_LOAD_A()                                                                                     \
// ... 841 lines not shown
    if ((uint32_t)rx >= c.prm.WC || (uint32_t)ry >= c.prm.WC) { atomicOr(c.prm.err, ERR_WINDOW); return -1; }
    const uint32_t pidx = ((uint32_t)ry >> 5) * c.prm.W + ((uint32_t)rx >> 5);
    int slot = c.dir[pidx];
    if (slot < 0) {
        if (c.count >= c.cap) { atomicOr(c.prm.err, ERR_DM_CAP); return -1; }
        slot = c.count++;
        c.dir[pidx] = (int16_t)slot;
    }
    const uint32_t ci = ((uint32_t)rx & 31u) | (((uint32_t)ry & 31u) << 5);
    uint64_t* w = c.mask + (size_t)slot * 16 + (ci >> 6);
    const uint64_t bit = 1ull << (ci & 63);
    const uint64_t cur = *w;
    if (!(cur & bit)) *w = cur | bit;
    return slot * 1024 + (int)ci;
}

__device__ inline void bf_push(BfCtx& c, bool to_lower, uint32_t prio, int rx, int ry)
{
    uint32_t& n = to_lower ? c.nl : c.nr;
    if (n >= c.prm.qcap) { atomicOr(c.prm.err, ERR_QUEUE); return; }
    if (to_lower) heap_push(c.lower, c.nl, q_entry(prio, rx, ry));
    else heap_push(c.raise, c.nr, q_entry(prio, rx, ry));
}

__device__ __noinline__ void bf_raise(BfCtx& c, int rx, int ry, int cur)
{
    const int DX[4] = {1, 0, -1, 0}, DY[4] = {0, 1, 0, -1};
    for (int i = 0; i < 4; ++i) {
        const int nx = rx + DX[i], ny = ry + DY[i];
        const int nc = bf_get(c, nx, ny);
        if (nc < 0) continue;
        const sv_t s = c.sv[nc];
        if ((s & SV_QUEUED) || !(s & SV_VALID)) continue;
        const uint32_t no = c.obs[nc];
        const int oc = bf_get(c, nx + obs_x(no), ny + obs_y(no));
        if (oc < 0) continue;
        if (!(c.sv[oc] & SV_VALID)) {
            bf_push(c, false, s & SV_SQMASK, nx, ny);
            c.sv[nc] = SV_QUEUED;
            c.obs[nc] = 0;
        } else {
            bf_push(c, true, s & SV_SQMASK, nx, ny);
            c.sv[nc] = s | SV_QUEUED;
        }
    }
    c.sv[cur] &= (sv_t)~SV_QUEUED;
}

__device__ __noinline__ void bf_lower(BfCtx& c, int rx, int ry, int cur)
{
    const sv_t s = c.sv[cur];
    if (!(s & SV_QUEUED)) return;
    const uint32_t co = c.obs[cur];
    const int cox = obs_x(co), coy = obs_y(co);
    const int obx = rx + cox, oby = ry + coy;
    const int DX[4] = {1, 0, -1, 0}, DY[4] = {0, 1, 0, -1};
    for (int i = 0; i < 4; ++i) {
        if (DX[i] * cox > 0 || DY[i] * coy > 0) continue;
        const int nx = rx + DX[i], ny = ry + DY[i];
        const int nc = bf_get(c, nx, ny);
        if (nc < 0) continue;
        const sv_t ns = c.sv[nc];
        const int qx = nx - obx, qy = ny - oby;
        const uint32_t new_sq = (uint32_t)(qx * qx + qy * qy);
        const uint32_t cmp = (ns & SV_VALID) ? (uint32_t)(ns & SV_SQMASK) : c.prm.max_sqdist;
        bool over = new_sq < cmp;
        if (!over && new_sq == (uint32_t)(ns & SV_SQMASK)) {
            const uint32_t nobs = c.obs[nc];
            const int oc = bf_get(c, nx + obs_x(nobs), ny + obs_y(nobs));
            if (oc >= 0) {
                const sv_t os = c.sv[oc];
                if (!(ns & SV_VALID) || !((os & SV_VALID) && (os & SV_SQMASK) == 0)) over = true;
            }
        }
        if (over) {
            bf_push(c, true, new_sq, nx, ny);
            c.sv[nc] = (sv_t)(SV_VALID | SV_QUEUED | (new_sq & SV_SQMASK));
            c.obs[nc] = pack_obs(obx - nx, oby - ny);
        }
    }
    c.sv[cur] &= (sv_t)~SV_QUEUED;
}

__global__ __launch_bounds__(UM_BLOCK) void k_brushfire_slow(DevParams prm, int first_particle)
{
    const int p = first_particle + blockIdx.x;
    if (prm.slow[p] == 0 || threadIdx.x != 0) return;
    const PV pv = pview(prm, p);
    BfCtx c{prm, pv.dm_dir, pv.dm_sv, pv.dm_obs, pv.dm_mask, prm.counts[2 * p], (int)pv.dm_cap,
            GlobalStore{prm.q_lower + (size_t)p * prm.qcap}, GlobalStore{prm.q_raise + (size_t)p * prm.qcap},
            prm.qsizes[2 * p], prm.qsizes[2 * p + 1], 0};
    while (c.nr > 0) {
        const uint64_t e = heap_pop(c.raise, c.nr);
        const int rx = q_rx(e), ry = q_ry(e);
        const int cur = bf_get(c, rx, ry);
        ++c.processed;
        if (cur < 0) continue;
        bf_raise(c, rx, ry, cur);
    }
    while (c.nl > 0) {
        const uint64_t e = heap_pop(c.lower, c.nl);
        const int rx = q_rx(e), ry = q_ry(e);
        const int cur = bf_get(c, rx, ry);
        ++c.processed;
        if (cur < 0) continue;
        const sv_t s = c.sv[cur];
        if (s & SV_VALID) {
            const uint32_t o = c.obs[cur];
            const int oc = bf_get(c, rx + obs_x(o), ry + obs_y(o));
            if (oc < 0) continue;
            if ((c.sv[oc] & SV_SQMASK) == 0) bf_lower(c, rx, ry, cur);
        }
    }
    prm.counts[2 * p] = c.count;
    prm.stats[4 * p + 3] += c.processed;
    prm.slow[p] = 0;
}

}
#include "lama_raycast_par.h"
#include "lama_raycast_patch.h"
#include "lama_brushfire_canon.h"
namespace lama_dev {

__global__ __launch_bounds__(UM_BLOCK) void k_dm_add_obstacles(DevParams prm, int p, const uint32_t* __restrict__ cells_xy, uint32_t n)
{
    __shared__ uint32_t lds_dc[DC_SIZE];
    const int lane = threadIdx.x;
    const PV pv = pview(prm, p);
    int16_t* dm_dir = pv.dm_dir;
    sv_t* dm_sv = pv.dm_sv;
    uint32_t* dm_obs = pv.dm_obs;
    uint64_t* dm_mask = pv.dm_mask;
    uint64_t* q_lower = prm.q_lower + (size_t)p * prm.qcap;
    int dm_count = prm.counts[2 * p];
    for (int k = lane; k < DC_SIZE; k += UM_BLOCK) lds_dc[k] = DC_EMPTY;
    __syncthreads();
    const DirCache dc{lds_dc, dm_dir, prm.W};
    uint32_t nl = 0;
    for (uint32_t base = 0; base < n; base += 64) {
        const uint32_t i = base + lane;
        const bool act = i < n;
        const uint32_t rx = (act ? cells_xy[2 * i] : 0u) - prm.wx0, ry = (act ? cells_xy[2 * i + 1] : 0u) - prm.wy0;
        const bool inwin = rx < prm.WC && ry < prm.WC;
        if (act && !inwin) atomicOr(prm.err, ERR_WINDOW);
        const bool want = act && inwin;
        const uint32_t pidx = (ry >> 5) * prm.W + (rx >> 5), ci = (rx & 31u) | ((ry & 31u) << 5);
        const int slot = coop_slot(dc, dm_dir, dm_count, (int)pv.dm_cap, want, pidx, ERR_DM_CAP, prm.err);
        bool first = true;
        for (int l = 0; l < 63; ++l) {
            const uint32_t ox = __shfl(rx, l, 64), oy = __shfl(ry, l, 64);
            const int ow = __shfl((int)want, l, 64);
            if (l < lane && ow && ox == rx && oy == ry) first = false;
        }
        bool push = false;
        if (want && slot >= 0) {
            atomicOr((unsigned long long*)(dm_mask + (size_t)slot * 16 + (ci >> 6)), 1ull << (ci & 63));
            const sv_t s = dm_sv[slot * 1024 + (int)ci];
            if (first && !((s & SV_VALID) && (s & SV_SQMASK) == 0)) {
                dm_sv[slot * 1024 + (int)ci] = (sv_t)(SV_VALID | SV_QUEUED);
                dm_obs[slot * 1024 + (int)ci] = 0;
                push = true;
            }
        }
        const unsigned long long pm = __ballot(push);
        const int cnt = __popcll(pm);
        if (nl + (uint32_t)cnt > prm.qcap) { if (lane == 0) atomicOr(prm.err, ERR_QUEUE); }
        else {
            if (push) q_lower[nl + (uint32_t)__popcll(pm & ((1ull << lane) - 1ull))] = q_entry(0, (int)rx, (int)ry);
            nl += (uint32_t)cnt;
        }
        __builtin_amdgcn_fence(__ATOMIC_SEQ_CST, "wavefront");
    }
    if (lane == 0) { prm.counts[2 * p] = dm_count; prm.qsizes[2 * p] = nl; prm.qsizes[2 * p + 1] = 0; }
}

__global__ __launch_bounds__(256) void k_shift_window(const int16_t* __restrict__ src, int16_t* __restrict__ dst, uint32_t Ws, uint32_t Wd, int dx, int dy,
                                                       size_t src_stride, size_t dst_stride, int32_t* err)
{
    const uint32_t p = blockIdx.x, idx = blockIdx.y * 256u + threadIdx.x;
    if (idx < Wd * Wd) {
        const int wy = (int)(idx / Wd), wx = (int)(idx % Wd);
        const int sx = wx + dx, sy = wy + dy;
        const bool in = sx >= 0 && sy >= 0 && sx < (int)Ws && sy < (int)Ws;
        dst[p * dst_stride + idx] = in ? src[p * src_stride + (size_t)sy * Ws + (size_t)sx] : (int16_t)-1;
    }
    if (idx < Ws * Ws) {
        const int wy = (int)(idx / Ws), wx = (int)(idx % Ws);
        const int tx = wx - dx, ty = wy - dy;
        if (!(tx >= 0 && ty >= 0 && tx < (int)Wd && ty < (int)Wd) && src[p * src_stride + idx] >= 0) atomicOr(err, ERR_WINDOW);
    }
}

__global__ __launch_bounds__(256) void k_update_cleanup(DevParams prm)
{
    const size_t WW = (size_t)prm.W * prm.W;
    const size_t k = (size_t)blockIdx.y * 256 + threadIdx.x;
    if (k >= WW) return;
    int16_t* a = prm.occ_dir + (size_t)blockIdx.x * WW + k;
// ... 208 lines not shown
```

iris_lama_amd/csrc/lama_raycast_par.h:

```cpp
#pragma once
#include "lama_dev.h"

namespace lama_dev {


constexpr int RP_BLOCK_SMALL = 256, RP_BLOCK_LARGE = 1024;
#ifdef LAMA_TEST_SMALL_QUEUES
constexpr int RP_SORT_SMALL = 512;
#else
constexpr int RP_SORT_SMALL = 2048;
#endif

__device__ inline int dir_alloc_one(int16_t* dir, uint32_t pidx, int32_t* count, int cap, int errbit, int32_t* err)
{
    uint32_t* w = reinterpret_cast<uint32_t*>(dir) + (pidx >> 1);
    const int sh = (int)(pidx & 1u) * 16;
    for (uint32_t spins = 0;; ++spins) {
        const uint32_t v = __hip_atomic_load(w, __ATOMIC_RELAXED, __HIP_MEMORY_SCOPE_AGENT);
        const int s = (int)(int16_t)((v >> sh) & 0xFFFFu);
        if (s >= 0) return s;
        if (s == -3) return -1;
        if (spins > (1u << 22)) { atomicOr(err, errbit); return -1; }
        if (s == -1) {
            const uint32_t locked = (v & ~(0xFFFFu << sh)) | (0xFFFEu << sh);
            if (atomicCAS(w, v, locked) == v) {
                int ns = atomicAdd(count, 1);
                if (ns >= cap) { atomicOr(err, errbit); ns = -3; }
                for (;;) {
                    const uint32_t cur = __hip_atomic_load(w, __ATOMIC_RELAXED, __HIP_MEMORY_SCOPE_AGENT);
                    const uint32_t nv = (cur & ~(0xFFFFu << sh)) | (((uint32_t)(uint16_t)(int16_t)ns) << sh);
                    if (atomicCAS(w, cur, nv) == cur) break;
                }
                return ns >= 0 ? ns : -1;
            }
        }
        __builtin_amdgcn_s_sleep(1);
    }
}
__device__ inline int dir_get_or_alloc(int16_t* dir, uint32_t pidx, int32_t* count, int cap, int errbit, int32_t* err)
{
    int s = dir[pidx];
    if (s >= 0) return s;
#ifdef LAMA_WAVE_SIM
    return dir_alloc_one(dir, pidx, count, cap, errbit, err);
#endif
    const int lane = (int)(threadIdx.x & 63u);
    const uint64_t key = ((uint64_t)(uintptr_t)dir << 20) ^ (uint64_t)pidx;
    int res = -1;
    bool pending = true;
    for (;;) {
        const unsigned long long m = __ballot(pending);
        if (m == 0ull) break;
        const int leader = __ffsll((long long)m) - 1;
        const uint32_t klo = (uint32_t)__builtin_amdgcn_readlane((int)(uint32_t)key, leader);
        const uint32_t khi = (uint32_t)__builtin_amdgcn_readlane((int)(uint32_t)(key >> 32), leader);
        int r = 0;
        if (lane == leader) r = dir_alloc_one(dir, pidx, count, cap, errbit, err);
        r = __builtin_amdgcn_readlane(r, leader);
        if (pending && (uint32_t)key == klo && (uint32_t)(key >> 32) == khi) { res = r; pending = false; }
    }
    return res;
}

struct BeamGeom {
    uint32_t mhx, mhy, msx, msy;
    uint32_t a0, a1, nn;
    int s0, s1;
    bool mark_hit;
    int steps;
    uint64_t magic;
};

__device__ inline BeamGeom beam_geometry(const DevParams& prm, const double* T, double px, double py, double pz)
{
    double hx = ((T[0] * px + T[1] * py) + T[2] * pz) + T[9];
    double hy = ((T[3] * px + T[4] * py) + T[5] * pz) + T[10];
    double hz = ((T[6] * px + T[7] * py) + T[8] * pz) + T[11];
    double sx = T[9], sy = T[10], sz = T[11];
    double abx = 0, aby = 0, abz = 0, ray_length = 1.0;
    BeamGeom g;
    g.mark_hit = true;
    if (prm.trunc_range > 0.0) {
        abx = hx - sx; aby = hy - sy; abz = hz - sz;
        ray_length = sqrt((abx * abx + aby * aby) + abz * abz);
        if (prm.trunc_range < ray_length) {
            hx = sx + abx / ray_length * prm.trunc_range;
            hy = sy + aby / ray_length * prm.trunc_range;
            hz = sz + abz / ray_length * prm.trunc_range;
            g.mark_hit = false;
        }
    }
    if (g.mark_hit && prm.trunc_ray > 0.0) {
        if (prm.trunc_range == 0.0) {
            abx = hx - sx; aby = hy - sy; abz = hz - sz;
            ray_length = sqrt((abx * abx + aby * aby) + abz * abz);
        }
        if (prm.trunc_ray < ray_length) {
            sx = hx - abx / ray_length * prm.trunc_ray;
            sy = hy - aby / ray_length * prm.trunc_ray;
            sz = hz - abz / ray_length * prm.trunc_ray;
        }
    }
    g.mhx = w2m(prm, hx); g.mhy = w2m(prm, hy);
    g.msx = w2m(prm, sx); g.msy = w2m(prm, sy);
    const uint32_t mhz = w2m(prm, hz), msz = w2m(prm, sz);
    const int64_t d0 = (int64_t)g.mhx - (int64_t)g.msx, d1 = (int64_t)g.mhy - (int64_t)g.msy, d2 = (int64_t)mhz - (int64_t)msz;
    const int64_t a0 = d0 < 0 ? -d0 : d0, a1 = d1 < 0 ? -d1 : d1, a2 = d2 < 0 ? -d2 : d2;
    const int64_t nn = a0 > a1 ? (a0 > a2 ? a0 : a2) : (a1 > a2 ? a1 : a2);
    g.s0 = d0 < 0 ? -1 : 1; g.s1 = d1 < 0 ? -1 : 1;
    g.a0 = (uint32_t)a0; g.a1 = (uint32_t)a1; g.nn = (uint32_t)(nn > 0xFFFFFFFFll ? 0xFFFFFFFFll : nn);
    g.steps = nn > 0 ? (int)g.nn - 1 : 0;
    if (nn >= 8192) g.steps = -1;
    g.magic = (1ull << 42) / (uint64_t)(2 * (nn > 0 && nn < 8192 ? nn : 1)) + 1ull;
    return g;
}

constexpr int ACT_SEQ_BITS = 26, ACT_XY_BITS = 15;
__device__ inline uint64_t act_key(uint32_t rx, uint32_t ry, uint32_t beam, uint32_t t)
{
    return ((uint64_t)((ry << ACT_XY_BITS) | rx) << ACT_SEQ_BITS) | (uint64_t)((beam << 13) | t);
}

__device__ inline void act_append(const DevParams& prm, int p, uint64_t key)
{
    const uint32_t k = atomicAdd(prm.act_count + p, 1u);
    if (k < prm.act_cap) prm.act[(size_t)p * prm.act_cap + k] = key;
    else atomicOr(prm.err, ERR_QUEUE);
}

struct RayRec;
struct RayChunk;
constexpr uint64_t RAY_BBOX_EMPTY = 0x0000FFFF0000FFFFull;
__device__ inline uint64_t ray_hits_record(const DevParams& prm, const BeamGeom& g, int p, int i, int n, RayRec* rec_out, uint64_t* bbox_out);
__device__ inline void ray_chunk_record(const DevParams& prm, const BeamGeom& g, uint64_t bb, int lane, RayChunk* chunks, size_t index);

template <class TAB>
__global__ __launch_bounds__(256) void k_ray_hits(DevParams prm, const double* __restrict__ pts, int n,
                                                   const double* __restrict__ tfs, int first_particle,
                                                   RayRec* __restrict__ rec_out = nullptr, uint64_t* __restrict__ bbox_out = nullptr, int alloc_only = 0,
                                                   RayChunk* __restrict__ chunk_out = nullptr, TAB tab = TAB())
{
    const int p = first_particle + blockIdx.x;
    if (p >= (int)prm.P) return;
    const int i = blockIdx.y * 256 + threadIdx.x;
    const int lane = threadIdx.x & 63;
    const bool live = i < n;
    const int ic = live ? i : n - 1;
    double T[12];
    if constexpr (std::is_same<TAB, TfTable>::value) {
        const int b = (int)blockIdx.x & (ARG_BLOCK - 1);
#pragma unroll
        for (int k = 0; k < 12; ++k) T[k] = tab.v[12 * b + k];
    } else uload_f64_w<12>(tfs + 12 * (size_t)p, T);
    const BeamGeom g = beam_geometry(prm, T, pts[3 * ic], pts[3 * ic + 1], pts[3 * ic + 2]);
    uint64_t bb = RAY_BBOX_EMPTY;
    if (rec_out && live) bb = ray_hits_record(prm, g, p, i, n, rec_out, bbox_out);
    if (chunk_out && (i & ~63) < n) ray_chunk_record(prm, g, bb, lane, chunk_out, (size_t)p * ((n + 63) / 64) + (i >> 6));
    if (live && g.steps < 0) atomicOr(prm.err, ERR_WINDOW);
    if (!alloc_only) {
        uint32_t st = (live && g.steps > 0) ? (uint32_t)g.steps : 0u;
        for (int off = 32; off > 0; off >>= 1) st += (uint32_t)__shfl_xor((int)st, off, 64);
        if (lane == 0 && st) atomicAdd((unsigned long long*)(prm.stats + 4 * p + 2), (unsigned long long)st);
    }
    bool hit = live && g.steps >= 0 && g.mark_hit;
    const uint32_t rx = g.mhx - prm.wx0, ry = g.mhy - prm.wy0;
    if (hit && (rx >= prm.WC || ry >= prm.WC)) { atomicOr(prm.err, ERR_WINDOW); hit = false; }
    const uint32_t pidx = (ry >> 5) * prm.W + (rx >> 5), ci = (rx & 31u) | ((ry & 31u) << 5);
    int slot = -1;
    const PV pv = pview(prm, p);
    if (hit) slot = dir_get_or_alloc(pv.occ_dir, pidx, prm.counts + 2 * p + 1, (int)pv.occ_cap, ERR_OCC_CAP, prm.err);
    hit = hit && slot >= 0 && !alloc_only;
    if (hit) atomicOr((unsigned long long*)(pv.occ_hit + (size_t)slot * 16 + (ci >> 6)), 1ull << (ci & 63));
    const unsigned long long hm = __ballot(hit);
    if (hm) {
        uint32_t base = 0;
        if (lane == (__ffsll((long long)hm) - 1)) base = atomicAdd(prm.act_count + p, (uint32_t)__popcll(hm));
        base = (uint32_t)__shfl((int)base, __ffsll((long long)hm) - 1, 64);
        if (hit) {
            const uint32_t k = base + (uint32_t)__popcll(hm & ((1ull << lane) - 1ull));
            if (k < prm.act_cap) prm.act[(size_t)p * prm.act_cap + k] = act_key(rx, ry, (uint32_t)i, 0u);
            else atomicOr(prm.err, ERR_QUEUE);
        }
    }
}

template <int RP_BLOCK>
__device__ inline void bitonic_sort(uint64_t* a, uint32_t m)
{
    for (uint32_t k = 2; k <= m; k <<= 1) {
        for (uint32_t j = k >> 1; j > 0; j >>= 1) {
            for (uint32_t i = threadIdx.x; i < m; i += RP_BLOCK) {
                const uint32_t ixj = i ^ j;
                if (ixj > i) {
                    const uint64_t x = a[i], y = a[ixj];
                    const bool up = (i & k) == 0;
                    if ((x > y) == up) { a[i] = y; a[ixj] = x; }
                }
            }
            __syncthreads();
        }
    }
}

template <int RP_BLOCK, int E>
__device__ inline void bitonic_sort_regs(uint64_t* a)
{
    constexpr uint32_t M = (uint32_t)RP_BLOCK * E;
    const uint32_t base = threadIdx.x * (uint32_t)E;
    uint64_t x[E];
#pragma unroll
    for (int r = 0; r < E; ++r) x[r] = a[base + r];
    for (uint32_t k = 2; k <= M; k <<= 1) {
        uint32_t j = k >> 1;
        for (; j >= 64u * E; j >>= 1) {
            __syncthreads();
#pragma unroll
            for (int r = 0; r < E; ++r) a[base + r] = x[r];
            __syncthreads();
            const uint32_t pb = base ^ j;
            const bool keep_min = ((base & j) == 0) == ((base & k) == 0);
#pragma unroll
            for (int r = 0; r < E; ++r) {
                const uint64_t y = a[pb + r];
                x[r] = ((y < x[r]) == keep_min) ? y : x[r];
            }
        }
        for (; j >= (uint32_t)E; j >>= 1) {
            const int lj = (int)(j / (uint32_t)E);
            const bool keep_min = ((base & j) == 0) == ((base & k) == 0);
#pragma unroll
            for (int r = 0; r < E; ++r) {
                const uint64_t y = __shfl_xor(x[r], lj, 64);
                x[r] = ((y < x[r]) == keep_min) ? y : x[r];
            }
        }
#pragma unroll
        for (int jr = E / 2; jr > 0; jr >>= 1) {
            if ((uint32_t)jr >= k) continue;
#pragma unroll
            for (int r = 0; r < E; ++r) {
                if (r & jr) continue;
                const bool up = ((base + (uint32_t)r) & k) == 0;
                const uint64_t lo = x[r], hi = x[r | jr];
                const bool sw = (lo > hi) == up;
                x[r] = sw ? hi : lo; x[r | jr] = sw ? lo : hi;
            }
        }
    }
    __syncthreads();
#pragma unroll
    for (int r = 0; r < E; ++r) a[base + r] = x[r];
    __syncthreads();
}

template <int RP_BLOCK>
__device__ inline void sort_keys(uint64_t* a, uint32_t m)
{
    if (m < (uint32_t)RP_BLOCK) { if (m > 1) bitonic_sort<RP_BLOCK>(a, m); }
    else if (m == (uint32_t)RP_BLOCK) bitonic_sort_regs<RP_BLOCK, 1>(a);
    else if (m == 2u * RP_BLOCK) bitonic_sort_regs<RP_BLOCK, 2>(a);
    else if (m == 4u * RP_BLOCK) bitonic_sort_regs<RP_BLOCK, 4>(a);
    else if (m == 8u * RP_BLOCK) bitonic_sort_regs<RP_BLOCK, 8>(a);
    else bitonic_sort<RP_BLOCK>(a, m);
}

template <int SORT_CAP, int EV_CAP>
struct ReplayLds {
    uint64_t keys[SORT_CAP];
    uint64_t ev[EV_CAP];
    uint32_t ev_n;
    uint32_t nadd, nrem;
};

template <int SORT_CAP, int EV_CAP, bool RESUME, int RP_BLOCK>
__device__ __forceinline__ void ray_replay_particle(const DevParams& prm, const int p, ReplayLds<SORT_CAP, EV_CAP>& sh)
{
    const uint32_t n = prm.act_count[p];
    if (RESUME && prm.slow[p] == 0) return;
    if (n > prm.act_cap) return;
    if (n > (uint32_t)SORT_CAP) {
        if (threadIdx.x == 0) {
            if (RESUME) atomicOr(prm.err, ERR_QUEUE);
            else { const uint32_t seg = prm.lane ? 3u : 1u; prm.slow[p] = 1; prm.slow_list[(size_t)seg * prm.P + atomicAdd(prm.slow_n + seg, 1u)] = (uint32_t)p; }
        }
        return;
    }
    const PV pv = pview_w(prm, p);
    int16_t* occ_dir = pv.occ_dir;
    int16_t* dm_dir = pv.dm_dir;
    uint32_t* occ = pv.occ;
    sv_t* dm_sv = pv.dm_sv;
    uint32_t* dm_obs = pv.dm_obs;
    uint64_t* q_lower = prm.q_lower + (size_t)p * prm.qcap;
    uint64_t* q_raise = prm.q_raise + (size_t)p * prm.qcap;

    uint32_t m = 1;
    while (m < n) m <<= 1;
    const uint64_t* src = prm.act + (size_t)p * prm.act_cap;
    for (uint32_t i = threadIdx.x; i < m; i += RP_BLOCK) sh.keys[i] = i < n ? src[i] : ~0ull;
    if (threadIdx.x == 0) { sh.ev_n = 0; sh.nadd = 0; sh.nrem = 0; }
    __syncthreads();
    sort_keys<RP_BLOCK>(sh.keys, m);

    for (uint32_t i = threadIdx.x; i < n; i += RP_BLOCK) {
        const uint64_t k0 = sh.keys[i];
        const uint32_t ck = (uint32_t)(k0 >> ACT_SEQ_BITS);
        if (i > 0 && (uint32_t)(sh.keys[i - 1] >> ACT_SEQ_BITS) == ck) continue;
        const uint32_t rx = ck & 32767u, ry = ck >> ACT_XY_BITS;
        const uint32_t pidx = (ry >> 5) * prm.W + (rx >> 5), ci = (rx & 31u) | ((ry & 31u) << 5);
        const uint64_t bit = 1ull << (ci & 63);
        const int slot = occ_dir[pidx];
        if (slot < 0) continue;
        uint32_t* cell = occ + (size_t)slot * 1024 + ci;
        const uint32_t v = *cell;
        uint32_t o = v & 0xFFFFu, vis = v >> 16;
        bool dm_loaded = false, dirty = false, had_hit = false;
        int dslot = -1;
        sv_t s = 0;
        for (uint32_t j = i; j < n; ++j) {
            const uint64_t kj = sh.keys[j];
            if ((uint32_t)(kj >> ACT_SEQ_BITS) != ck) break;
            const uint32_t seq = (uint32_t)(kj & 0x3FFFFFFu);
            const bool is_hit = (seq & 8191u) == 0;
            bool changed;
            if (is_hit) {
                had_hit = true;
                const bool occupied = vis != 0 && 4u * o > vis;
                o = (o + 1) & 0xFFFFu; vis = (vis + 1) & 0xFFFFu;
                changed = !occupied && (vis != 0 && 4u * o > vis);
            } else {
                const bool was_free = vis != 0 && 4u * o < vis;
                vis = (vis + 1) & 0xFFFFu;
                changed = !was_free && (vis != 0 && 4u * o < vis);
            }
            if (vis == 0) atomicOr((unsigned long long*)(pv.occ_mask + (size_t)slot * 16 + (ci >> 6)), (unsigned long long)bit);
            if (!changed) continue;
            if (!dm_loaded) {
                dslot = dir_get_or_alloc(dm_dir, pidx, prm.counts + 2 * p, (int)pv.dm_cap, ERR_DM_CAP, prm.err);
                dm_loaded = true;
                if (dslot >= 0) {
                    atomicOr((unsigned long long*)(pv.dm_mask + (size_t)dslot * 16 + (ci >> 6)), (unsigned long long)bit);
                    s = dm_sv[dslot * 1024 + (int)ci];
                }
            }
            if (dslot < 0) continue;
            const bool is_obstacle = (s & SV_VALID) && (s & SV_SQMASK) == 0;
            bool emit = false;
            if (is_hit && !is_obstacle) { s = (sv_t)(SV_VALID | SV_QUEUED); emit = true; }
            if (!is_hit && is_obstacle) { s = SV_QUEUED; emit = true; }
            if (emit) {
                dirty = true;
                const uint32_t e = atomicAdd(&sh.ev_n, 1u);
                if (e < (uint32_t)EV_CAP) sh.ev[e] = ((uint64_t)seq << 32) | ((uint64_t)(is_hit ? 1u : 0u) << 31) | ck;
                else atomicOr(prm.err, ERR_QUEUE);
            }
        }
        *cell = o | (vis << 16);
        if (dirty) { dm_sv[dslot * 1024 + (int)ci] = s; dm_obs[dslot * 1024 + (int)ci] = 0; }
        if (had_hit) atomicAnd((unsigned long long*)(pv.occ_hit + (size_t)slot * 16 + (ci >> 6)), ~(unsigned long long)bit);
    }
    __syncthreads();

    const uint32_t ne = sh.ev_n < (uint32_t)EV_CAP ? sh.ev_n : (uint32_t)EV_CAP;
    uint32_t me = 1;
    while (me < ne) me <<= 1;
    for (uint32_t i = ne + threadIdx.x; i < me; i += RP_BLOCK) sh.ev[i] = ~0ull;
    __syncthreads();
    if (me > 1) bitonic_sort<RP_BLOCK>(sh.ev, me);
    if (threadIdx.x < 64) {
        const int lane = threadIdx.x;
        uint32_t nadd = 0, nrem = 0;
        for (uint32_t base = 0; base < ne; base += 64) {
            const uint32_t i = base + lane;
            const bool act = i < ne;
            const uint64_t e = act ? sh.ev[i] : 0ull;
            const bool is_add = act && ((e >> 31) & 1ull);
            const bool is_rem = act && !is_add;
            const unsigned long long ma = __ballot(is_add), mr = __ballot(is_rem);
            const uint32_t ck = (uint32_t)(e & 0x3FFFFFFFu);
            const int rx = (int)(ck & 32767u), ry = (int)(ck >> ACT_XY_BITS);
            const unsigned long long lt = (1ull << lane) - 1ull;
            if (is_add) { const uint32_t k = nadd + (uint32_t)__popcll(ma & lt); if (k < prm.qcap) q_lower[k] = q_entry(0, rx, ry); else atomicOr(prm.err, ERR_QUEUE); }
            if (is_rem) { const uint32_t k = nrem + (uint32_t)__popcll(mr & lt); if (k < prm.qcap) q_raise[k] = q_entry(0, rx, ry); else atomicOr(prm.err, ERR_QUEUE); }
            nadd += (uint32_t)__popcll(ma);
            nrem += (uint32_t)__popcll(mr);
        }
        if (lane == 0) {
            prm.qsizes[2 * p] = nadd < prm.qcap ? nadd : prm.qcap;
            prm.qsizes[2 * p + 1] = nrem < prm.qcap ? nrem : prm.qcap;
            prm.act_count[p] = 0;
            prm.slow[p] = 0;
        }
    }
}


template <int SORT_CAP, int EV_CAP, bool RESUME, int RP_BLOCK>
__global__ __launch_bounds__(RP_BLOCK) void k_ray_replay(DevParams prm, int first_particle)
{
    __shared__ ReplayLds<SORT_CAP, EV_CAP> sh;
    if (map_update_aborted(prm)) return;
    if (!RESUME) {
        const int p = lane_particle(prm, first_particle, (int)blockIdx.x);
        if (p >= 0) ray_replay_particle<SORT_CAP, EV_CAP, RESUME, RP_BLOCK>(prm, p, sh);
        return;
    }
    const uint32_t seg = prm.lane ? 3u : 1u;
    const uint32_t n = uload_u32(prm.slow_n + seg);
    for (uint32_t i = blockIdx.x; i < n; i += gridDim.x) {
        ray_replay_particle<SORT_CAP, EV_CAP, RESUME, RP_BLOCK>(prm, (int)uload_u32(prm.slow_list + (size_t)seg * prm.P + i), sh);
        __syncthreads();
    }
}

}
```

iris_lama_amd/csrc/lama_raycast_patch.h:

```cpp
#pragma once
#include "lama_raycast_par.h"

namespace lama_dev {

struct RayRec {
    uint32_t msx, msy;
    uint32_t a01;
    uint32_t nnf;
    uint64_t magic;
};
struct RayChunk {
    int32_t cwx, cwy;
    int32_t ccwx, ccwy;
    uint64_t bbox;
    uint32_t sxy;
    uint32_t cone;
};

__device__ inline RayRec ray_rec(const BeamGeom& g)
{
    RayRec r;
    r.msx = g.msx; r.msy = g.msy;
    r.a01 = (g.a0 & 0xFFFFu) | ((g.a1 & 0xFFFFu) << 16);
    r.nnf = (g.nn & 0xFFFFu) | (g.s0 < 0 ? 1u << 16 : 0u) | (g.s1 < 0 ? 1u << 17 : 0u) | (g.steps > 0 ? 1u << 18 : 0u);
    r.magic = g.magic;
    return r;
}
__device__ __forceinline__ void ray_cell(const RayRec& r, uint32_t wx0, uint32_t wy0, uint32_t t, uint32_t& rx, uint32_t& ry)
{
    const uint32_t a0 = r.a01 & 0xFFFFu, a1 = r.a01 >> 16, nn = r.nnf & 0xFFFFu;
    const uint32_t st0 = (uint32_t)(((uint64_t)(2u * t * a0 + nn) * r.magic) >> 42);
    const uint32_t st1 = (uint32_t)(((uint64_t)(2u * t * a1 + nn) * r.magic) >> 42);
    const uint32_t cx = (r.nnf & (1u << 16)) ? r.msx - st0 : r.msx + st0;
    const uint32_t cy = (r.nnf & (1u << 17)) ? r.msy - st1 : r.msy + st1;
    rx = cx - wx0; ry = cy - wy0;
}

__device__ __forceinline__ bool ray_axis_range(int m, bool neg, uint32_t a, uint32_t nn, int lo, uint32_t steps, uint32_t& t_lo, uint32_t& t_hi)
{
    int ka = neg ? m - (lo + 31) : lo - m, kb = neg ? m - lo : lo + 31 - m;
    if (ka < 0) ka = 0;
    if (kb > (int)a) kb = (int)a;
    if (ka > kb) return false;
    t_lo = 1u; t_hi = steps;
    if (a == 0u) return true;
    const uint32_t d = 2u * a;
    if (ka > 0) t_lo = (2u * nn * (uint32_t)ka - nn + d - 1u) / d;
    if (kb < (int)a) t_hi = (2u * nn * (uint32_t)(kb + 1) - nn + d - 1u) / d - 1u;
    if (t_lo < 1u) t_lo = 1u;
    if (t_hi > steps) t_hi = steps;
    return t_lo <= t_hi;
}

__device__ inline uint64_t ray_hits_record(const DevParams& prm, const BeamGeom& g, int p, int i, int n, RayRec* rec_out, uint64_t* bbox_out)
{
    RayRec r = ray_rec(g);
    uint64_t bb = RAY_BBOX_EMPTY;
    bool ok = g.steps > 0;
    if (ok) {
        const int64_t xa = (int64_t)g.msx - (int64_t)prm.wx0, ya = (int64_t)g.msy - (int64_t)prm.wy0;
        const int64_t xb = xa + (int64_t)g.s0 * (int64_t)g.a0, yb = ya + (int64_t)g.s1 * (int64_t)g.a1;
        const int64_t x0 = xa < xb ? xa : xb, x1 = xa < xb ? xb : xa, y0 = ya < yb ? ya : yb, y1 = ya < yb ? yb : ya;
        if (x0 < 0 || y0 < 0 || x1 >= (int64_t)prm.WC || y1 >= (int64_t)prm.WC) { atomicOr(prm.err, ERR_WINDOW); ok = false; }
        else bb = (uint64_t)x0 | ((uint64_t)x1 << 16) | ((uint64_t)y0 << 32) | ((uint64_t)y1 << 48);
    }
    if (!ok) r.nnf &= ~(1u << 18);
    rec_out[(size_t)p * n + i] = r;
    bbox_out[(size_t)p * n + i] = bb;
    return bb;
}

__device__ inline void ray_chunk_record(const DevParams& prm, const BeamGeom& g, uint64_t bb, int lane, RayChunk* chunks, size_t index)
{
    const bool val = bb != RAY_BBOX_EMPTY;
    const unsigned long long vm = __ballot(val);
    uint32_t x0 = (uint32_t)(bb & 0xFFFFu), x1 = (uint32_t)((bb >> 16) & 0xFFFFu), y0 = (uint32_t)((bb >> 32) & 0xFFFFu), y1 = (uint32_t)(bb >> 48);
    for (int off = 32; off > 0; off >>= 1) {
        const uint32_t ox0 = (uint32_t)__shfl_xor((int)x0, off, 64), ox1 = (uint32_t)__shfl_xor((int)x1, off, 64);
        const uint32_t oy0 = (uint32_t)__shfl_xor((int)y0, off, 64), oy1 = (uint32_t)__shfl_xor((int)y1, off, 64);
        x0 = ox0 < x0 ? ox0 : x0; x1 = ox1 > x1 ? ox1 : x1; y0 = oy0 < y0 ? oy0 : y0; y1 = oy1 > y1 ? oy1 : y1;
    }
    const int lf = vm ? __ffsll((long long)vm) - 1 : 0, ll = vm ? 63 - __clzll((long long)vm) : 0;
    const int dx = g.s0 < 0 ? -(int)g.a0 : (int)g.a0, dy = g.s1 < 0 ? -(int)g.a1 : (int)g.a1;
    const int sx = (int)(g.msx - prm.wx0), sy = (int)(g.msy - prm.wy0);
    const int fx = __shfl(dx, lf, 64), fy = __shfl(dy, lf, 64), lx = __shfl(dx, ll, 64), ly = __shfl(dy, ll, 64);
    const int fsx = __shfl(sx, lf, 64), fsy = __shfl(sy, lf, 64);
    const int c_f = fx * dy - fy * dx, c_l = dx * ly - dy * lx;
    const bool front = fx * dx + fy * dy > 0 && lx * dx + ly * dy > 0 && sx == fsx && sy == fsy;
    const bool all_ccw = __ballot(val && !(front && c_f >= 0 && c_l >= 0)) == 0ull;
    const bool all_cw = __ballot(val && !(front && c_f <= 0 && c_l <= 0)) == 0ull;
    if (lane == 0) {
        RayChunk c;
        c.bbox = vm ? ((uint64_t)x0 | ((uint64_t)x1 << 16) | ((uint64_t)y0 << 32) | ((uint64_t)y1 << 48)) : RAY_BBOX_EMPTY;
        c.sxy = ((uint32_t)fsx & 0xFFFFu) | ((uint32_t)fsy << 16);
        c.cone = (vm && (all_ccw || all_cw)) ? 1u : 0u;
        c.cwx = all_ccw ? fx : lx; c.cwy = all_ccw ? fy : ly;
        c.ccwx = all_ccw ? lx : fx; c.ccwy = all_ccw ? ly : fy;
        chunks[index] = c;
    }
}

__global__ __launch_bounds__(256) void k_ray_alloc_walk(DevParams prm, const RayRec* __restrict__ recs, int n, int first_particle, int RW_SEG)
{
    const int p = first_particle + blockIdx.x;
    const int g = blockIdx.y * 256 + threadIdx.x;
    const int i = g / RW_SEG, seg = g % RW_SEG;
    if (i >= n || p >= (int)prm.P) return;
    const RayRec r = recs[(size_t)p * n + i];
    if (!(r.nnf & (1u << 18))) return;
    const uint32_t steps = (r.nnf & 0xFFFFu) - 1u;
    const uint32_t t0 = 1u + (uint32_t)(((uint64_t)steps * (uint32_t)seg) / RW_SEG), t1 = (uint32_t)(((uint64_t)steps * (uint32_t)(seg + 1)) / RW_SEG);
    const PV pv = pview(prm, p);
    int16_t* occ_dir = pv.occ_dir;
    if (t0 > t1) return;
    const uint32_t a0 = r.a01 & 0xFFFFu, a1 = r.a01 >> 16, nn = r.nnf & 0xFFFFu;
    const uint32_t k0 = (uint32_t)(((uint64_t)(2u * t0 * a0 + nn) * r.magic) >> 42), k1 = (uint32_t)(((uint64_t)(2u * t0 * a1 + nn) * r.magic) >> 42);
    const bool neg0 = (r.nnf >> 16) & 1u, neg1 = (r.nnf >> 17) & 1u;
    const uint32_t bx = r.msx - prm.wx0, by = r.msy - prm.wy0;
    const uint32_t rx = neg0 ? bx - k0 : bx + k0, ry = neg1 ? by - k1 : by + k1;
    uint32_t X = rx >> 5, Y = ry >> 5;
    uint32_t kx = neg0 ? k0 + (rx & 31u) + 1u : k0 + 32u - (rx & 31u), ky = neg1 ? k1 + (ry & 31u) + 1u : k1 + 32u - (ry & 31u);
    auto step_of = [nn](uint32_t k, uint32_t a) { return k > a ? 0xFFFFFFFFu : (2u * nn * k - nn + 2u * a - 1u) / (2u * a); };
    uint32_t tx = step_of(kx, a0), ty = step_of(ky, a1);
    (void)dir_get_or_alloc(occ_dir, Y * prm.W + X, prm.counts + 2 * p + 1, (int)pv.occ_cap, ERR_OCC_CAP, prm.err);
    for (;;) {
        const uint32_t t = tx < ty ? tx : ty;
        if (t > t1) break;
        if (tx == t) { X = neg0 ? X - 1u : X + 1u; kx += 32u; tx = step_of(kx, a0); }
        if (ty == t) { Y = neg1 ? Y - 1u : Y + 1u; ky += 32u; ty = step_of(ky, a1); }
        (void)dir_get_or_alloc(occ_dir, Y * prm.W + X, prm.counts + 2 * p + 1, (int)pv.occ_cap, ERR_OCC_CAP, prm.err);
    }
}

__device__ inline int imin(int a, int b) { return a < b ? a : b; }
__device__ inline int imax(int a, int b) { return a > b ? a : b; }
constexpr int RD_MARK_SIDE = 256;
constexpr int RD_MARK_WORDS = RD_MARK_SIDE * RD_MARK_SIDE / 32;

template <class TAB>
__global__ __launch_bounds__(256) void k_occ_reverse_dir(DevParams prm, int first_particle,
                                                          const double* __restrict__ tfs , int reach_cells, int guard_off,
                                                          uint32_t row0, uint32_t row1, TAB tab)
{
    __shared__ uint32_t mark[RD_MARK_WORDS];
    __shared__ uint32_t need_s;
    const int p = first_particle + blockIdx.x;
    const uint32_t W = prm.W;
    const int tid = threadIdx.x, r = (int)prm.guard_r;
    const PV pv = pview_w(prm, p);
    const int16_t* occ_dir = pv.occ_dir;
    const int16_t* dm_dir = pv.dm_dir;
    double stx, sty;
    if constexpr (std::is_same<TAB, TfTable>::value) { const int tb = (int)blockIdx.x & (ARG_BLOCK - 1); stx = tab.v[12 * tb + 9]; sty = tab.v[12 * tb + 10]; }
    else { stx = uload_f64(tfs + 12 * (size_t)p + 9); sty = uload_f64(tfs + 12 * (size_t)p + 10); }
    const int scx = (int)(w2m(prm, stx) - prm.wx0), scy = (int)(w2m(prm, sty) - prm.wy0);
    const int bx0 = imax((scx - reach_cells) >> 5, 0), bx1 = imin((scx + reach_cells) >> 5, (int)W - 1);
    const int by0 = imax((scy - reach_cells) >> 5, 0), by1 = imin((scy + reach_cells) >> 5, (int)W - 1);
    const int mx0 = imax(bx0 - r, 0), my0 = imax(by0 - r, 0), mw = imin(bx1 + r, (int)W - 1) - mx0 + 1, mh = imin(by1 + r, (int)W - 1) - my0 + 1;
    const bool bounded = mw > 0 && mh > 0 && mw <= RD_MARK_SIDE && mh <= RD_MARK_SIDE;
    const uint32_t nbits = bounded ? (uint32_t)(mw * mh) : 0u;
    for (uint32_t i = tid; i < (nbits + 31u) / 32u; i += 256u) mark[i] = 0;
    if (tid == 0) need_s = 0;
    __syncthreads();
    const uint32_t w_end = (row1 < W ? row1 + 1u : W) * W;
    for (uint32_t w0 = row0 * W + (uint32_t)tid * 8u; w0 < w_end; w0 += 256u * 8u) {
        const uint4 q = *reinterpret_cast<const uint4*>(occ_dir + w0);
        if ((q.x & q.y & q.z & q.w) == 0xFFFFFFFFu) continue;
        const uint32_t ww[4] = {q.x, q.y, q.z, q.w};
        const int wy = (int)(w0 / W), x0 = (int)(w0 % W);
#pragma unroll
        for (int k = 0; k < 8; ++k) {
            const int slot = (int)(int16_t)((ww[k >> 1] >> ((k & 1) * 16)) & 0xFFFFu);
            if (slot < 0) continue;
            pv.rev[slot] = (int32_t)(w0 + (uint32_t)k);
            if (!bounded || x0 + k < bx0 || x0 + k > bx1 || wy < by0 || wy > by1) continue;
            for (int dy = -r; dy <= r; ++dy)
                for (int dx = -r; dx <= r; ++dx) {
                    const int x = x0 + k + dx - mx0, y = wy + dy - my0;
                    if ((uint32_t)x < (uint32_t)mw && (uint32_t)y < (uint32_t)mh) { const uint32_t n = (uint32_t)y * (uint32_t)mw + (uint32_t)x; atomicOr(&mark[n >> 5], 1u << (n & 31u)); }
                }
        }
    }
    __syncthreads();
    uint32_t need = 0;
    for (uint32_t n = (uint32_t)tid; n < nbits; n += 256u) {
        if (!((mark[n >> 5] >> (n & 31u)) & 1u)) continue;
        const uint32_t wx = (uint32_t)mx0 + n % (uint32_t)mw, wy = (uint32_t)my0 + n / (uint32_t)mw;
        if (dm_dir[wy * W + wx] < 0) ++need;
    }
    if (need) atomicAdd(&need_s, need);
    __syncthreads();
    const bool tiled = !bounded && mw > 0 && mh > 0;
    if (tiled) {
        for (int ty = my0; ty < my0 + mh; ty += RD_MARK_SIDE)
            for (int tx = mx0; tx < mx0 + mw; tx += RD_MARK_SIDE) {
                const int tw = imin(RD_MARK_SIDE, mx0 + mw - tx), th = imin(RD_MARK_SIDE, my0 + mh - ty);
                const uint32_t tbits = (uint32_t)(tw * th);
                for (uint32_t i = tid; i < (tbits + 31u) / 32u; i += 256u) mark[i] = 0;
                __syncthreads();
                const int ry0 = imax(ty - r, by0), ry1 = imin(ty + th - 1 + r, by1);
                const int rx0 = imax(tx - r, bx0), rx1 = imin(tx + tw - 1 + r, bx1);
                const int nx = rx1 - rx0 + 1, nrow = ry1 - ry0 + 1;
                for (int i = tid; nx > 0 && i < nx * nrow; i += 256) {
                    const int ox = rx0 + i % nx, oy = ry0 + i / nx;
                    if (occ_dir[(uint32_t)oy * W + (uint32_t)ox] < 0) continue;
                    for (int dy = -r; dy <= r; ++dy)
                        for (int dx = -r; dx <= r; ++dx) {
                            const int x = ox + dx - tx, y = oy + dy - ty;
                            if ((uint32_t)x < (uint32_t)tw && (uint32_t)y < (uint32_t)th) { const uint32_t n = (uint32_t)y * (uint32_t)tw + (uint32_t)x; atomicOr(&mark[n >> 5], 1u << (n & 31u)); }
                        }
                }
                __syncthreads();
                uint32_t tneed = 0;
                for (uint32_t i = tid; i < (tbits + 31u) / 32u; i += 256u) {
                    uint32_t m = mark[i];
                    while (m) {
                        const uint32_t n = i * 32u + (uint32_t)(__ffs((int)m) - 1);
                        const uint32_t wx = (uint32_t)tx + n % (uint32_t)tw, wy = (uint32_t)ty + n / (uint32_t)tw;
                        if (dm_dir[wy * W + wx] < 0) ++tneed;
                        m &= m - 1u;
                    }
                }
                if (tneed) atomicAdd(&need_s, tneed);
                __syncthreads();
            }
    }
    if (tid == 0) prm.guard[p] = (bounded || tiled) ? need_s : 0u;
    if (tid == 0 && (bounded || tiled) && !guard_off && (uint64_t)prm.counts[2 * p] + need_s > pv.dm_cap) atomicOr(prm.err, ERR_DM_CAP);
}

#ifdef LAMA_PROFILE_RAY
#ifdef LAMA_PROFILE_RAY_COUNT
#define RPC(k, v) atomicAdd((unsigned long long*)(prm.dbg + 16 * (size_t)prm.P + (k)), (unsigned long long)(v))
#else
#define RPC(k, v) do {} while (0)
#endif
#define RPT_T(k) do { if (tid == 0) { const uint64_t t_ = __builtin_readcyclecounter(); tacc[(k) - 8] += t_ - tprev; tprev = t_; } } while (0)
#else
#define RPC(k, v) do {} while (0)
#define RPT_T(k) do {} while (0)
#endif
constexpr int RPT_CHUNK = 256;
#ifndef LAMA_RPT_WALK
#define LAMA_RPT_WALK 4
#endif
constexpr int RPT_WALK = LAMA_RPT_WALK;

__global__ __launch_bounds__(256, 6) void k_ray_patches(DevParams prm, const RayRec* __restrict__ recs, const uint64_t* __restrict__ bbox,
                                                      const RayChunk* __restrict__ chunks, int n, int first_particle)
{
    static_assert(RPT_CHUNK == 256, "one candidate beam per thread and round");
    __shared__ uint32_t cnt[1024];
    __shared__ RayRec lrec[RPT_CHUNK];
    __shared__ uint32_t lbt[RPT_CHUNK];
    __shared__ uint16_t lbeam[RPT_CHUNK];
    __shared__ uint32_t actw[32], newm[32], wrapm[32];
    __shared__ uint32_t list_n[2];
    const int p = lane_particle(prm, first_particle, (int)blockIdx.x);
    const int tid = threadIdx.x, lane = tid & 63, wave = tid >> 6;
    if (map_update_aborted(prm)) { if (blockIdx.x == 0 && blockIdx.y == 0 && tid == 0) atomicOr(prm.err, ERR_CLEAN_ABORT); return; }
    if (p < 0) return;
    const int count = prm.counts[2 * p + 1];
    const PVOcc pv = pview_occ_w(prm, p);
    uint32_t* occ = pv.occ;
    const RayRec* prec = recs + (size_t)p * n;
    const uint64_t* pbb = bbox + (size_t)p * n;
    const int nck = (n + 63) / 64;
    RayChunk ck;
    ck.bbox = RAY_BBOX_EMPTY; ck.cone = 0; ck.cwx = ck.cwy = ck.ccwx = ck.ccwy = 0; ck.sxy = 0;
    if (lane < nck) ck = chunks[(size_t)p * nck + lane];
    if (tid < 2) list_n[tid] = 0;
    int slot = blockIdx.y;
    uint32_t pidx_next = slot < count ? (uint32_t)pv.rev[slot] : 0u;
    uint32_t par = 0;
#ifdef LAMA_PROFILE_RAY
    uint64_t tacc[8] = {0, 0, 0, 0, 0, 0, 0, 0}, tprev = 0;
#endif
    __syncthreads();
    for (; slot < count; slot += gridDim.y) {
        const uint32_t pidx = pidx_next;
        if (slot + (int)gridDim.y < count) pidx_next = (uint32_t)pv.rev[slot + gridDim.y];
        const int px = (int)((pidx % prm.W) * 32u), py = (int)((pidx / prm.W) * 32u);
#ifdef LAMA_PROFILE_RAY
        tprev = __builtin_readcyclecounter();
        ++tacc[5];
        if (tid == 0) RPC(0, 1);
#endif
        bool keep = false;
        if (lane < nck) {
            const int x0 = (int)(ck.bbox & 0xFFFFu), x1 = (int)((ck.bbox >> 16) & 0xFFFFu), y0 = (int)((ck.bbox >> 32) & 0xFFFFu), y1 = (int)(ck.bbox >> 48);
            keep = !(x1 < px || x0 > px + 31 || y1 < py || y0 > py + 31);
            if (keep && ck.cone) {
                const int sx = (int)(ck.sxy & 0xFFFFu), sy = (int)(ck.sxy >> 16);
                const int ax = px - 1 - sx, bx = px + 32 - sx, ay = py - 1 - sy, by = py + 32 - sy;
                const int a00 = ck.cwx * ay - ck.cwy * ax, a10 = ck.cwx * ay - ck.cwy * bx, a01 = ck.cwx * by - ck.cwy * ax, a11 = ck.cwx * by - ck.cwy * bx;
                const int b00 = ck.ccwx * ay - ck.ccwy * ax, b10 = ck.ccwx * ay - ck.ccwy * bx, b01 = ck.ccwx * by - ck.ccwy * ax, b11 = ck.ccwx * by - ck.ccwy * bx;
                if ((a00 < 0 && a10 < 0 && a01 < 0 && a11 < 0) || (b00 > 0 && b10 > 0 && b01 > 0 && b11 > 0)) keep = false;
            }
        }
        const unsigned long long km = __ballot(keep);
        const int ncand = __popcll(km) * 64;
        if (tid == 0) RPC(2, __popcll(km));
        if (km == 0ull) continue;
        uint32_t v[4];
        uint64_t hw[4];
        const uint64_t* hitw = pv.occ_hit + (size_t)slot * 16;
#pragma unroll
        for (int j = 0; j < 4; ++j) { v[j] = occ[(size_t)slot * 1024 + tid + 256 * j]; hw[j] = hitw[wave + 4 * j]; }
        bool has_act = false;
        for (int c0 = 0; c0 == 0 || c0 < ncand; c0 += RPT_CHUNK, par ^= 1u) {
            const int jc = (c0 >> 6) + wave;
// ... 117 lines not shown
```

Before: 17860 particle-scans/s.

## Fuse ray front kernels per particle and merge replay/brushfire resume passes

Adds a per-particle k_ray_front kernel that runs ray hits, allocation walk and occupancy reverse-direction scan in one block, separated by block barriers with thread fences, replacing three launches. It also adds k_update_resume, which handles the replay and brushfire resume/slow paths in a single kernel with a shared LDS union, replacing separate resume launches. The aim is to cut launch overhead and inter-kernel gaps for small particle counts. The cost is that each particle now gets one block instead of a 2D grid across beams, so parallelism drops, and the resume kernel uses a large LDS footprint.

```diff
diff --git a/iris_lama_amd/csrc/lama_dev.h b/iris_lama_amd/csrc/lama_dev.h
--- a/iris_lama_amd/csrc/lama_dev.h
+++ b/iris_lama_amd/csrc/lama_dev.h
@@ -55,6 +55,8 @@
     int32_t* rev;
     uint64_t r1;
 };
+
+constexpr uint32_t SLOW_BRUSHFIRE = 1u, SLOW_REPLAY = 2u;
 
 struct DevParams {
     uint32_t P;
diff --git a/iris_lama_amd/csrc/lama_hip.hip b/iris_lama_amd/csrc/lama_hip.hip
--- a/iris_lama_amd/csrc/lama_hip.hip
+++ b/iris_lama_amd/csrc/lama_hip.hip
@@ -256,6 +256,8 @@
     StepGroup grp[MAX_STEP_GROUPS];
     Stream stream4;
     uint32_t step_groups = 1;
+    bool fused_update = true;
+    uint32_t front_block = 1024;
     uint32_t groups_ran = 0;
     std::vector<int32_t> deferred_idx; bool resample_deferred = false;
     bool groups_busy = false;
@@ -440,8 +442,8 @@
 
 void apply_update_status(lama_hip_ctx* c, const StatusView& v, uint32_t first, uint32_t count, uint64_t* chain)
 {
-    uint32_t sn[5]; std::memcpy(sn, v.slow_n, sizeof(sn));
-    c->ctr.brushfire_handovers += sn[0]; c->ctr.replay_handovers += sn[1] + sn[3]; c->ctr.brushfire_routed += sn[2] + sn[4]; c->ctr.brushfire_early += sn[4];
+    uint32_t sn[6]; std::memcpy(sn, v.slow_n, sizeof(sn));
+    c->ctr.brushfire_handovers += sn[0] + sn[5]; c->ctr.replay_handovers += sn[1] + sn[3]; c->ctr.brushfire_routed += sn[2] + sn[4]; c->ctr.brushfire_early += sn[4];
     c->early_candidates = sn[2] + sn[4];
     c->h_guard.resize(c->P);
     std::memcpy(&c->h_guard[v.base], v.guard, sizeof(uint32_t) * v.n);
@@ -936,6 +938,8 @@
     bool sequential = false, guarded = true, canon = false, two_waves = false, route = false, early_lane = false;
     bool prev_routed = false; uint32_t host_n = 0;
     uint32_t route_places = 0; unsigned gy = 0, resume_grid = 0; bool replay_large = true;
+    bool fused = false;
+    bool fused_resume = false;
 };
 
 static bool parallel_raycast_ruled_out(const lama_hip_ctx* c, uint32_t n)
@@ -954,6 +958,7 @@
     u.gy = 4u;
 #endif
     u.replay_large = count <= 512; u.resume_grid = std::min<unsigned>(count, 256u);
+    u.fused = g && c->fused_update; u.fused_resume = u.fused && u.two_waves;
     if (g) return u;
     u.sequential = parallel_raycast_ruled_out(c, n) || wrap_sequential;
     u.guarded = c->cfg.ray_rule == 0;
@@ -1040,11 +1045,13 @@
         if (e == hipSuccess) e = c->d_rchunk.alloc((size_t)c->P * ((n + 63) / 64));
         if (e != hipSuccess) { c->d_rrec.reset(); return hip_fail(c, e, "ray buffers"); }
     }
-    const dim3 hits_grid(xcd_grid(c, first, count), (n + 255) / 256);
-    hipLaunchKernelGGL(k_ray_hits<Tab>, hits_grid, dim3(256), 0, u.s, u.prm, u.d_pts, (int)n, d_tfs, (int)first,
-                       (lama_dev::RayRec*)c->d_rrec, (uint64_t*)c->d_rbbox, alloc_only, (lama_dev::RayChunk*)c->d_rchunk, tab);
     const int rw_seg = count <= 64 ? 4 : 1;
-    hipLaunchKernelGGL(k_ray_alloc_walk, dim3(xcd_grid(c, first, count), (n * rw_seg + 255) / 256), dim3(256), 0, u.s, u.prm, (const lama_dev::RayRec*)c->d_rrec, (int)n, (int)first, rw_seg);
+    if (!u.fused) {
+        const dim3 hits_grid(xcd_grid(c, first, count), (n + 255) / 256);
+        hipLaunchKernelGGL(k_ray_hits<Tab>, hits_grid, dim3(256), 0, u.s, u.prm, u.d_pts, (int)n, d_tfs, (int)first,
+                           (lama_dev::RayRec*)c->d_rrec, (uint64_t*)c->d_rbbox, alloc_only, (lama_dev::RayChunk*)c->d_rchunk, tab);
+        hipLaunchKernelGGL(k_ray_alloc_walk, dim3(xcd_grid(c, first, count), (n * rw_seg + 255) / 256), dim3(256), 0, u.s, u.prm, (const lama_dev::RayRec*)c->d_rrec, (int)n, (int)first, rw_seg);
+    }
     double far = c->scan_reach;
     if (c->cfg.truncated_range > 0.0) far = std::min(far, c->cfg.truncated_range);
     const int reach_cells = (int)std::ceil(far * c->scale) + 2;
@@ -1054,7 +1061,15 @@
         const int64_t lo = std::min(std::max(c->mby0 - oy, (int64_t)0), W - 1), hi = std::min(std::max(c->mby1 - oy, (int64_t)0), W - 1);
         if (hi >= lo) { row0 = (uint32_t)lo; row1 = (uint32_t)hi; }
     }
-    hipLaunchKernelGGL(k_occ_reverse_dir<Tab>, dim3(count), dim3(256), 0, u.s, u.prm, (int)first, d_tfs, reach_cells, c->unguarded_retry ? 1 : 0, row0, row1, tab);
+    if (u.fused && c->front_block == 256)
+        hipLaunchKernelGGL((k_ray_front<Tab, 256>), dim3(count), dim3(256), 0, u.s, u.prm, u.d_pts, (int)n, d_tfs, (int)first,
+                           (lama_dev::RayRec*)c->d_rrec, (uint64_t*)c->d_rbbox, (lama_dev::RayChunk*)c->d_rchunk, alloc_only, rw_seg,
+                           reach_cells, c->unguarded_retry ? 1 : 0, row0, row1, tab);
+    else if (u.fused)
+        hipLaunchKernelGGL((k_ray_front<Tab, RF_BLOCK>), dim3(count), dim3(RF_BLOCK), 0, u.s, u.prm, u.d_pts, (int)n, d_tfs, (int)first,
+                           (lama_dev::RayRec*)c->d_rrec, (uint64_t*)c->d_rbbox, (lama_dev::RayChunk*)c->d_rchunk, alloc_only, rw_seg,
+                           reach_cells, c->unguarded_retry ? 1 : 0, row0, row1, tab);
+    else hipLaunchKernelGGL(k_occ_reverse_dir<Tab>, dim3(count), dim3(256), 0, u.s, u.prm, (int)first, d_tfs, reach_cells, c->unguarded_retry ? 1 : 0, row0, row1, tab);
     return LAMA_HIP_OK;
 }
 int32_t launch_allocation_phase(lama_hip_ctx* c, const UpdatePlan& u, int alloc_only) { return u.tf_by_value ? launch_allocation_phase(c, u, alloc_only, u.tab) : launch_allocation_phase(c, u, alloc_only, lama_dev::NoTable()); }
@@ -1091,7 +1106,7 @@
                        (const uint64_t*)c->d_rbbox, (const lama_dev::RayChunk*)c->d_rchunk, (int)u.n, first);
     if (u.replay_large) {
         hipLaunchKernelGGL((k_ray_replay<RP_SORT_SMALL, RP_SORT_SMALL, false, RP_BLOCK_LARGE>), dim3(u.count), dim3(RP_BLOCK_LARGE), 0, u.s, prm, first);
-        hipLaunchKernelGGL((k_ray_replay<8192, 8192, true, RP_BLOCK_LARGE>), dim3(u.resume_grid), dim3(RP_BLOCK_LARGE), 0, u.s, prm, first);
+        if (!u.fused_resume) hipLaunchKernelGGL((k_ray_replay<8192, 8192, true, RP_BLOCK_LARGE>), dim3(u.resume_grid), dim3(RP_BLOCK_LARGE), 0, u.s, prm, first);
     } else {
         hipLaunchKernelGGL((k_ray_replay<RP_SORT_SMALL, RP_SORT_SMALL, false, RP_BLOCK_SMALL>), dim3(u.count), dim3(RP_BLOCK_SMALL), 0, u.s, prm, first);
         hipLaunchKernelGGL((k_ray_replay<8192, 8192, true, RP_BLOCK_SMALL>), dim3(u.resume_grid), dim3(RP_BLOCK_SMALL), 0, u.s, prm, first);
@@ -1115,6 +1130,10 @@
         HIPCHK(c, hipStreamWaitEvent(c->stream, c->ev_heavy, 0));
     } else if (u.two_waves) hipLaunchKernelGGL((k_brushfire<LQ_SMALL, RQ_SMALL, false, true>), dim3(u.count), dim3(2 * UM_BLOCK), 0, u.s, prm, first, 0);
     else hipLaunchKernelGGL((k_brushfire<LQ_SMALL, RQ_SMALL, false, false>), dim3(u.count), dim3(UM_BLOCK), 0, u.s, prm, first, 0);
+    if (u.fused_resume) {
+        hipLaunchKernelGGL(k_update_resume, dim3(u.resume_grid), dim3(lama_dev::UR_BLOCK), 0, u.s, prm);
+        return LAMA_HIP_OK;
+    }
     if (u.two_waves) hipLaunchKernelGGL((k_brushfire<LQ_BIG, RQ_BIG, true, true>), dim3(u.resume_grid), dim3(2 * UM_BLOCK), 0, u.s, prm, first, 0);
     else hipLaunchKernelGGL((k_brushfire<LQ_BIG, RQ_BIG, true, false>), dim3(u.resume_grid), dim3(UM_BLOCK), 0, u.s, prm, first, 0);
     if (u.early_lane) HIPCHK(c, hipStreamWaitEvent(c->stream, c->ev_early, 0));
@@ -1533,6 +1552,8 @@
         }
         if (c->P >= c->route_min_count) G = 1;
         c->step_groups = G;
+        if (const char* fu = std::getenv("LAMA_HIP_FUSED_UPDATE")) c->fused_update = !(fu[0] == '0' && fu[1] == 0);
+        if (const char* fb = std::getenv("LAMA_HIP_FRONT_BLOCK")) c->front_block = (uint32_t)std::atoi(fb);
         if (G > 1) {
             if (G > 3 && hipStreamCreate(&c->stream4.h)) return LAMA_HIP_E_HIP;
             const hipStream_t ss[MAX_STEP_GROUPS] = {c->stream, c->stream2, c->stream3, c->stream4};
@@ -2546,7 +2567,7 @@
     HIPCHK(c, hipMemcpyAsync(d_cells, cells_xy, sizeof(uint32_t) * 2 * (size_t)n, hipMemcpyHostToDevice, c->stream));
     DevParams prm = make_params(c);
     if (n > c->cfg.queue_capacity) return fail(c, LAMA_HIP_E_CAPACITY, "more obstacle cells than cfg.queue_capacity");
-    HIPCHK(c, hipMemsetAsync(c->d_slow_n, 0, 5 * sizeof(uint32_t), c->stream));
+    HIPCHK(c, hipMemsetAsync(c->d_slow_n, 0, 6 * sizeof(uint32_t), c->stream));
     hipLaunchKernelGGL(k_dm_add_obstacles, dim3(1), dim3(UM_BLOCK), 0, c->stream, prm, (int)particle, d_cells, n);
     hipLaunchKernelGGL((k_brushfire<LQ_SMALL, RQ_SMALL, false, true>), dim3(1), dim3(2 * UM_BLOCK), 0, c->stream, prm, (int)particle, 0);
     hipLaunchKernelGGL((k_brushfire<LQ_BIG, RQ_BIG, true, true>), dim3(1), dim3(2 * UM_BLOCK), 0, c->stream, prm, (int)particle, 0);
diff --git a/iris_lama_amd/csrc/lama_kernels.h b/iris_lama_amd/csrc/lama_kernels.h
--- a/iris_lama_amd/csrc/lama_kernels.h
+++ b/iris_lama_amd/csrc/lama_kernels.h
@@ -1027,7 +1027,7 @@
 
 __device__ __forceinline__ void bf_hand_over(const DevParams& prm, int p, bool from_resume)
 {
-    prm.slow[p] = 1;
+    prm.slow[p] = SLOW_BRUSHFIRE;
     if (!from_resume) prm.slow_list[atomicAdd(prm.slow_n, 1u)] = (uint32_t)p;
 }
 
@@ -1036,7 +1036,7 @@
 {
     const int p = __builtin_amdgcn_readfirstlane(p_any);
     if (!RESUME && prm.heavy != nullptr && (prm.heavy[p] != 0 || (prm.early != nullptr && prm.early[p] != 0))) return;
-    const uint32_t handed = RESUME ? prm.slow[p] : 1u;
+    const uint32_t handed = RESUME ? prm.slow[p] : uload_u32(prm.slow + p);
     const int lane = threadIdx.x & 63;
     const int tid = threadIdx.x, nthreads = TW ? 2 * UM_BLOCK : UM_BLOCK;
     const PV pv = pview_w(prm, p);
@@ -1051,7 +1051,7 @@
     const uint64_t nlr = uload_u64(prm.qsizes + 2 * p);
     uint32_t nl = (uint32_t)nlr, nr = (uint32_t)(nlr >> 32);
     if (RESUME && TW) __syncthreads(); else LAMA_LOCKSTEP();
-    if (RESUME && handed == 0) return;
+    if (RESUME ? handed == 0 : handed == SLOW_REPLAY) return;
     if (tid == 0) prm.slow[p] = 0;
     if (nl == 0 && nr == 0) return;
     if (nl + 4 > (uint32_t)LQ_LDS || nr + 4 > (uint32_t)RQ_LDS) { if (tid == 0) bf_hand_over(prm, p, RESUME); return; }
@@ -2059,10 +2059,9 @@
     c.sv[cur] &= (sv_t)~SV_QUEUED;
 }
 
-__global__ __launch_bounds__(UM_BLOCK) void k_brushfire_slow(DevParams prm, int first_particle)
-{
-    const int p = first_particle + blockIdx.x;
-    if (prm.slow[p] == 0 || threadIdx.x != 0) return;
+__device__ inline void bf_slow_particle(const DevParams& prm, int p)
+{
+    if (prm.slow[p] == 0) return;
     const PV pv = pview(prm, p);
     BfCtx c{prm, pv.dm_dir, pv.dm_sv, pv.dm_obs, pv.dm_mask, prm.counts[2 * p], (int)pv.dm_cap,
             GlobalStore{prm.q_lower + (size_t)p * prm.qcap}, GlobalStore{prm.q_raise + (size_t)p * prm.qcap},
@@ -2092,6 +2091,11 @@
     prm.counts[2 * p] = c.count;
     prm.stats[4 * p + 3] += c.processed;
     prm.slow[p] = 0;
+}
+
+__global__ __launch_bounds__(UM_BLOCK) void k_brushfire_slow(DevParams prm, int first_particle)
+{
+    if (threadIdx.x == 0) bf_slow_particle(prm, first_particle + blockIdx.x);
 }
 
 }
diff --git a/iris_lama_amd/csrc/lama_raycast_par.h b/iris_lama_amd/csrc/lama_raycast_par.h
--- a/iris_lama_amd/csrc/lama_raycast_par.h
+++ b/iris_lama_amd/csrc/lama_raycast_par.h
@@ -5,6 +5,7 @@
 
 
 constexpr int RP_BLOCK_SMALL = 256, RP_BLOCK_LARGE = 1024;
+constexpr int RF_BLOCK = 1024;
 #ifdef LAMA_TEST_SMALL_QUEUES
 constexpr int RP_SORT_SMALL = 512;
 #else
@@ -135,23 +136,21 @@
 __device__ inline void ray_chunk_record(const DevParams& prm, const BeamGeom& g, uint64_t bb, int lane, RayChunk* chunks, size_t index);
 
 template <class TAB>
-__global__ __launch_bounds__(256) void k_ray_hits(DevParams prm, const double* __restrict__ pts, int n,
-                                                   const double* __restrict__ tfs, int first_particle,
-                                                   RayRec* __restrict__ rec_out = nullptr, uint64_t* __restrict__ bbox_out = nullptr, int alloc_only = 0,
-                                                   RayChunk* __restrict__ chunk_out = nullptr, TAB tab = TAB())
-{
-    const int p = first_particle + blockIdx.x;
-    if (p >= (int)prm.P) return;
-    const int i = blockIdx.y * 256 + threadIdx.x;
+__device__ __forceinline__ void scan_tf_of_block(const TAB& tab, const double* tfs, int p, double (&T)[12])
+{
+    if constexpr (std::is_same<TAB, TfTable>::value) {
+        const int b = (int)blockIdx.x & (ARG_BLOCK - 1);
+#pragma unroll
+        for (int k = 0; k < 12; ++k) T[k] = tab.v[12 * b + k];
+    } else uload_f64_w<12>(tfs + 12 * (size_t)p, T);
+}
+
+__device__ __forceinline__ void ray_hits_beam(const DevParams& prm, const PV& pv, const double (&T)[12], const double* __restrict__ pts, int n, int p, int i,
+                                              RayRec* rec_out, uint64_t* bbox_out, int alloc_only, RayChunk* chunk_out)
+{
     const int lane = threadIdx.x & 63;
     const bool live = i < n;
     const int ic = live ? i : n - 1;
-    double T[12];
-    if constexpr (std::is_same<TAB, TfTable>::value) {
-        const int b = (int)blockIdx.x & (ARG_BLOCK - 1);
-#pragma unroll
-        for (int k = 0; k < 12; ++k) T[k] = tab.v[12 * b + k];
-    } else uload_f64_w<12>(tfs + 12 * (size_t)p, T);
     const BeamGeom g = beam_geometry(prm, T, pts[3 * ic], pts[3 * ic + 1], pts[3 * ic + 2]);
     uint64_t bb = RAY_BBOX_EMPTY;
     if (rec_out && live) bb = ray_hits_record(prm, g, p, i, n, rec_out, bbox_out);
@@ -167,7 +166,6 @@
     if (hit && (rx >= prm.WC || ry >= prm.WC)) { atomicOr(prm.err, ERR_WINDOW); hit = false; }
     const uint32_t pidx = (ry >> 5) * prm.W + (rx >> 5), ci = (rx & 31u) | ((ry & 31u) << 5);
     int slot = -1;
-    const PV pv = pview(prm, p);
     if (hit) slot = dir_get_or_alloc(pv.occ_dir, pidx, prm.counts + 2 * p + 1, (int)pv.occ_cap, ERR_OCC_CAP, prm.err);
     hit = hit && slot >= 0 && !alloc_only;
     if (hit) atomicOr((unsigned long long*)(pv.occ_hit + (size_t)slot * 16 + (ci >> 6)), 1ull << (ci & 63));
@@ -184,6 +182,19 @@
     }
 }
 
+template <class TAB>
+__global__ __launch_bounds__(256) void k_ray_hits(DevParams prm, const double* __restrict__ pts, int n,
+                                                   const double* __restrict__ tfs, int first_particle,
+                                                   RayRec* __restrict__ rec_out = nullptr, uint64_t* __restrict__ bbox_out = nullptr, int alloc_only = 0,
+                                                   RayChunk* __restrict__ chunk_out = nullptr, TAB tab = TAB())
+{
+    const int p = first_particle + blockIdx.x;
+    if (p >= (int)prm.P) return;
+    double T[12];
+    scan_tf_of_block(tab, tfs, p, T);
+    ray_hits_beam(prm, pview(prm, p), T, pts, n, p, blockIdx.y * 256 + threadIdx.x, rec_out, bbox_out, alloc_only, chunk_out);
+}
+
 template <int RP_BLOCK>
 __device__ inline void bitonic_sort(uint64_t* a, uint32_t m)
 {
@@ -273,17 +284,17 @@
 };
 
 template <int SORT_CAP, int EV_CAP, bool RESUME, int RP_BLOCK>
-__device__ __forceinline__ void ray_replay_particle(const DevParams& prm, const int p, ReplayLds<SORT_CAP, EV_CAP>& sh)
+__device__ __forceinline__ bool ray_replay_particle(const DevParams& prm, const int p, ReplayLds<SORT_CAP, EV_CAP>& sh)
 {
     const uint32_t n = prm.act_count[p];
-    if (RESUME && prm.slow[p] == 0) return;
-    if (n > prm.act_cap) return;
+    if (RESUME && prm.slow[p] == 0) return false;
+    if (n > prm.act_cap) return false;
     if (n > (uint32_t)SORT_CAP) {
         if (threadIdx.x == 0) {
             if (RESUME) atomicOr(prm.err, ERR_QUEUE);
-            else { const uint32_t seg = prm.lane ? 3u : 1u; prm.slow[p] = 1; prm.slow_list[(size_t)seg * prm.P + atomicAdd(prm.slow_n + seg, 1u)] = (uint32_t)p; }
-        }
-        return;
+            else { const uint32_t seg = prm.lane ? 3u : 1u; prm.slow[p] = SLOW_REPLAY; prm.slow_list[(size_t)seg * prm.P + atomicAdd(prm.slow_n + seg, 1u)] = (uint32_t)p; }
+        }
+        return false;
     }
     const PV pv = pview_w(prm, p);
     int16_t* occ_dir = pv.occ_dir;
@@ -392,6 +403,7 @@
             prm.slow[p] = 0;
         }
     }
+    return true;
 }
 
 
@@ -413,4 +425,42 @@
     }
 }
 
-}
+constexpr int UR_BLOCK = 2 * UM_BLOCK;
+union UpdateResumeLds {
+    ReplayLds<8192, 8192> replay;
+    BfLds<LQ_SMALL, RQ_SMALL> bf_first;
+    BfLds<LQ_BIG, RQ_BIG> bf;
+};
+__device__ __forceinline__ void update_resume_barrier()
+{
+    __threadfence();
+    __syncthreads();
+    __threadfence();
+}
+__device__ __forceinline__ void update_resume_brushfire(const DevParams& prm, int p, BfLds<LQ_BIG, RQ_BIG>& sh)
+{
+    bf_particle<LQ_BIG, RQ_BIG, true, true>(prm, p, sh);
+    update_resume_barrier();
+    if (threadIdx.x == 0) bf_slow_particle(prm, p);
+    update_resume_barrier();
+}
+__global__ __launch_bounds__(UR_BLOCK) void k_update_resume(DevParams prm)
+{
+    __shared__ UpdateResumeLds sh;
+    const uint32_t n_replay = uload_u32(prm.slow_n + 1), n_bf = uload_u32(prm.slow_n);
+    if (n_replay == 0 && n_bf == 0) return;
+    if (map_update_aborted(prm)) return;
+    DevParams late = prm; late.slow_n = prm.slow_n + 5; late.slow_list = prm.slow_list + 2 * (size_t)prm.P;
+    for (uint32_t i = blockIdx.x; i < n_replay; i += gridDim.x) {
+        const int p = (int)uload_u32(prm.slow_list + (size_t)prm.P + i);
+        const bool replayed = ray_replay_particle<8192, 8192, true, UR_BLOCK>(prm, p, sh.replay);
+        update_resume_barrier();
+        if (!replayed) { if (threadIdx.x == 0) prm.slow[p] = 0; continue; }
+        bf_particle<LQ_SMALL, RQ_SMALL, false, true>(late, p, sh.bf_first);
+        update_resume_barrier();
+        update_resume_brushfire(prm, p, sh.bf);
+    }
+    for (uint32_t i = blockIdx.x; i < n_bf; i += gridDim.x) update_resume_brushfire(prm, (int)uload_u32(prm.slow_list + i), sh.bf);
+}
+
+}
diff --git a/iris_lama_amd/csrc/lama_raycast_patch.h b/iris_lama_amd/csrc/lama_raycast_patch.h
--- a/iris_lama_amd/csrc/lama_raycast_patch.h
+++ b/iris_lama_amd/csrc/lama_raycast_patch.h
@@ -100,17 +100,14 @@
     }
 }
 
-__global__ __launch_bounds__(256) void k_ray_alloc_walk(DevParams prm, const RayRec* __restrict__ recs, int n, int first_particle, int RW_SEG)
-{
-    const int p = first_particle + blockIdx.x;
-    const int g = blockIdx.y * 256 + threadIdx.x;
+__device__ __forceinline__ void ray_alloc_walk_thread(const DevParams& prm, const PV& pv, const RayRec* recs, int n, int p, int g, int RW_SEG)
+{
     const int i = g / RW_SEG, seg = g % RW_SEG;
-    if (i >= n || p >= (int)prm.P) return;
+    if (i >= n) return;
     const RayRec r = recs[(size_t)p * n + i];
     if (!(r.nnf & (1u << 18))) return;
     const uint32_t steps = (r.nnf & 0xFFFFu) - 1u;
     const uint32_t t0 = 1u + (uint32_t)(((uint64_t)steps * (uint32_t)seg) / RW_SEG), t1 = (uint32_t)(((uint64_t)steps * (uint32_t)(seg + 1)) / RW_SEG);
-    const PV pv = pview(prm, p);
     int16_t* occ_dir = pv.occ_dir;
     if (t0 > t1) return;
     const uint32_t a0 = r.a01 & 0xFFFFu, a1 = r.a01 >> 16, nn = r.nnf & 0xFFFFu;
@@ -132,38 +129,38 @@
     }
 }
 
+__global__ __launch_bounds__(256) void k_ray_alloc_walk(DevParams prm, const RayRec* __restrict__ recs, int n, int first_particle, int RW_SEG)
+{
+    const int p = first_particle + blockIdx.x;
+    const int g = blockIdx.y * 256 + threadIdx.x;
+    if (g / RW_SEG >= n || p >= (int)prm.P) return;
+    ray_alloc_walk_thread(prm, pview(prm, p), recs, n, p, g, RW_SEG);
+}
+
 __device__ inline int imin(int a, int b) { return a < b ? a : b; }
 __device__ inline int imax(int a, int b) { return a > b ? a : b; }
 constexpr int RD_MARK_SIDE = 256;
 constexpr int RD_MARK_WORDS = RD_MARK_SIDE * RD_MARK_SIDE / 32;
 
-template <class TAB>
-__global__ __launch_bounds__(256) void k_occ_reverse_dir(DevParams prm, int first_particle,
-                                                          const double* __restrict__ tfs , int reach_cells, int guard_off,
-                                                          uint32_t row0, uint32_t row1, TAB tab)
-{
-    __shared__ uint32_t mark[RD_MARK_WORDS];
-    __shared__ uint32_t need_s;
-    const int p = first_particle + blockIdx.x;
+template <int BLOCK>
+__device__ __forceinline__ void occ_reverse_dir_particle(const DevParams& prm, const PV& pv, int p, double stx, double sty, int reach_cells, int guard_off,
+                                                         uint32_t row0, uint32_t row1, uint32_t* mark, uint32_t& need_s)
+{
     const uint32_t W = prm.W;
     const int tid = threadIdx.x, r = (int)prm.guard_r;
-    const PV pv = pview_w(prm, p);
     const int16_t* occ_dir = pv.occ_dir;
     const int16_t* dm_dir = pv.dm_dir;
-    double stx, sty;
-    if constexpr (std::is_same<TAB, TfTable>::value) { const int tb = (int)blockIdx.x & (ARG_BLOCK - 1); stx = tab.v[12 * tb + 9]; sty = tab.v[12 * tb + 10]; }
-    else { stx = uload_f64(tfs + 12 * (size_t)p + 9); sty = uload_f64(tfs + 12 * (size_t)p + 10); }
     const int scx = (int)(w2m(prm, stx) - prm.wx0), scy = (int)(w2m(prm, sty) - prm.wy0);
     const int bx0 = imax((scx - reach_cells) >> 5, 0), bx1 = imin((scx + reach_cells) >> 5, (int)W - 1);
     const int by0 = imax((scy - reach_cells) >> 5, 0), by1 = imin((scy + reach_cells) >> 5, (int)W - 1);
     const int mx0 = imax(bx0 - r, 0), my0 = imax(by0 - r, 0), mw = imin(bx1 + r, (int)W - 1) - mx0 + 1, mh = imin(by1 + r, (int)W - 1) - my0 + 1;
     const bool bounded = mw > 0 && mh > 0 && mw <= RD_MARK_SIDE && mh <= RD_MARK_SIDE;
     const uint32_t nbits = bounded ? (uint32_t)(mw * mh) : 0u;
-    for (uint32_t i = tid; i < (nbits + 31u) / 32u; i += 256u) mark[i] = 0;
+    for (uint32_t i = tid; i < (nbits + 31u) / 32u; i += (uint32_t)BLOCK) mark[i] = 0;
     if (tid == 0) need_s = 0;
     __syncthreads();
     const uint32_t w_end = (row1 < W ? row1 + 1u : W) * W;
-    for (uint32_t w0 = row0 * W + (uint32_t)tid * 8u; w0 < w_end; w0 += 256u * 8u) {
+    for (uint32_t w0 = row0 * W + (uint32_t)tid * 8u; w0 < w_end; w0 += (uint32_t)BLOCK * 8u) {
         const uint4 q = *reinterpret_cast<const uint4*>(occ_dir + w0);
         if ((q.x & q.y & q.z & q.w) == 0xFFFFFFFFu) continue;
         const uint32_t ww[4] = {q.x, q.y, q.z, q.w};
@@ -183,7 +180,7 @@
     }
     __syncthreads();
     uint32_t need = 0;
-    for (uint32_t n = (uint32_t)tid; n < nbits; n += 256u) {
+    for (uint32_t n = (uint32_t)tid; n < nbits; n += (uint32_t)BLOCK) {
         if (!((mark[n >> 5] >> (n & 31u)) & 1u)) continue;
         const uint32_t wx = (uint32_t)mx0 + n % (uint32_t)mw, wy = (uint32_t)my0 + n / (uint32_t)mw;
         if (dm_dir[wy * W + wx] < 0) ++need;
@@ -196,12 +193,12 @@
             for (int tx = mx0; tx < mx0 + mw; tx += RD_MARK_SIDE) {
                 const int tw = imin(RD_MARK_SIDE, mx0 + mw - tx), th = imin(RD_MARK_SIDE, my0 + mh - ty);
                 const uint32_t tbits = (uint32_t)(tw * th);
-                for (uint32_t i = tid; i < (tbits + 31u) / 32u; i += 256u) mark[i] = 0;
+                for (uint32_t i = tid; i < (tbits + 31u) / 32u; i += (uint32_t)BLOCK) mark[i] = 0;
                 __syncthreads();
                 const int ry0 = imax(ty - r, by0), ry1 = imin(ty + th - 1 + r, by1);
                 const int rx0 = imax(tx - r, bx0), rx1 = imin(tx + tw - 1 + r, bx1);
                 const int nx = rx1 - rx0 + 1, nrow = ry1 - ry0 + 1;
-                for (int i = tid; nx > 0 && i < nx * nrow; i += 256) {
+                for (int i = tid; nx > 0 && i < nx * nrow; i += BLOCK) {
                     const int ox = rx0 + i % nx, oy = ry0 + i / nx;
                     if (occ_dir[(uint32_t)oy * W + (uint32_t)ox] < 0) continue;
                     for (int dy = -r; dy <= r; ++dy)
@@ -212,7 +209,7 @@
                 }
                 __syncthreads();
                 uint32_t tneed = 0;
-                for (uint32_t i = tid; i < (tbits + 31u) / 32u; i += 256u) {
+                for (uint32_t i = tid; i < (tbits + 31u) / 32u; i += (uint32_t)BLOCK) {
                     uint32_t m = mark[i];
                     while (m) {
                         const uint32_t n = i * 32u + (uint32_t)(__ffs((int)m) - 1);
@@ -227,6 +224,57 @@
     }
     if (tid == 0) prm.guard[p] = (bounded || tiled) ? need_s : 0u;
     if (tid == 0 && (bounded || tiled) && !guard_off && (uint64_t)prm.counts[2 * p] + need_s > pv.dm_cap) atomicOr(prm.err, ERR_DM_CAP);
+}
+
+template <class TAB>
+__global__ __launch_bounds__(256) void k_occ_reverse_dir(DevParams prm, int first_particle,
+                                                          const double* __restrict__ tfs , int reach_cells, int guard_off,
+                                                          uint32_t row0, uint32_t row1, TAB tab)
+{
+    __shared__ uint32_t mark[RD_MARK_WORDS];
+    __shared__ uint32_t need_s;
+    const int p = first_particle + blockIdx.x;
+    double stx, sty;
+    if constexpr (std::is_same<TAB, TfTable>::value) { const int tb = (int)blockIdx.x & (ARG_BLOCK - 1); stx = tab.v[12 * tb + 9]; sty = tab.v[12 * tb + 10]; }
+    else { stx = uload_f64(tfs + 12 * (size_t)p + 9); sty = uload_f64(tfs + 12 * (size_t)p + 10); }
+    occ_reverse_dir_particle<256>(prm, pview_w(prm, p), p, stx, sty, reach_cells, guard_off, row0, row1, mark, need_s);
+}
+
+__device__ __forceinline__ void front_phase_barrier()
+{
+    __threadfence();
+    __syncthreads();
+    __threadfence();
+}
+
+template <class TAB, int BLOCK>
+__global__ __launch_bounds__(BLOCK) void k_ray_front(DevParams prm, const double* __restrict__ pts, int n, const double* tfs, int first_particle,
+                                                      RayRec* rec, uint64_t* bbox, RayChunk* chunks, int alloc_only, int RW_SEG,
+                                                      int reach_cells, int guard_off, uint32_t row0, uint32_t row1, TAB tab)
+{
+    static_assert(BLOCK % 64 == 0, "a wave of the first phase is 64 consecutive beams (the chunk cone)");
+    __shared__ uint32_t mark[RD_MARK_WORDS];
+    __shared__ uint32_t need_s;
+    const int p = first_particle + blockIdx.x;
+    const int tid = threadIdx.x;
+    const PV pv = pview_w(prm, p);
+    double T[12];
+    scan_tf_of_block(tab, tfs, p, T);
+#ifndef LAMA_WAVE_SIM
+#pragma unroll
+    for (int k = 0; k < 12; ++k) {
+        const uint64_t w = (uint64_t)__double_as_longlong(T[k]);
+        T[k] = __longlong_as_double((long long)(((uint64_t)(uint32_t)__builtin_amdgcn_readfirstlane((int)(uint32_t)(w >> 32)) << 32) | (uint32_t)__builtin_amdgcn_readfirstlane((int)(uint32_t)w)));
+    }
+#endif
+    for (int base = 0; base < n; base += BLOCK) {
+        const int i = base + tid;
+        if ((i & ~63) < n) ray_hits_beam(prm, pv, T, pts, n, p, i, rec, bbox, alloc_only, chunks);
+    }
+    front_phase_barrier();
+    for (int g = tid; g < n * RW_SEG; g += BLOCK) ray_alloc_walk_thread(prm, pv, rec, n, p, g, RW_SEG);
+    front_phase_barrier();
+    occ_reverse_dir_particle<BLOCK>(prm, pv, p, T[9], T[10], reach_cells, guard_off, row0, row1, mark, need_s);
 }
 
 #ifdef LAMA_PROFILE_RAY
```

New measurement: 17350 particle-scans/s. -2.8%, worse.
